# TSultanov/cfd-demo

Hardware: AMD Instinct MI355X
Metric: cell-updates/s (Poisson iter) + ms/timestep, 4096² grid, 1/2/4/8 GPU (higher is better)
Workload: dtype f32

## Files before the change

### cfd-demo_amd/csrc/cfd_correct.h

```cpp
#pragma once
#include "cfd_device.h"

namespace cfd {
namespace {

template <int SP>
__device__ __forceinline__ float u_corr(const Geom &g, float us, float pr, float pw, float dt, int i) {
    return i >= g.nx - 7 ? us - sdiv<SP>(dt * (pr - pw), g.dx, g.r_dx)
                         : us - dt * sdiv<SP>(pr - pw, g.dx, g.r_dx);
}

template <int SP>
__device__ __forceinline__ float v_corr(const Geom &g, float vs, float pt, float pb, float dt) {
    return vs - dt * sdiv<SP>(pt - pb, g.dy, g.r_dy);
}
template <int SP>
__device__ __forceinline__ void v_corr4(const Geom &g, const float4 &vs, const float4 &pt,
                                        const float4 &pb, float dt, float4 &o) {
    o.x = v_corr<SP>(g, vs.x, pt.x, pb.x, dt);
    o.y = v_corr<SP>(g, vs.y, pt.y, pb.y, dt);
    o.z = v_corr<SP>(g, vs.z, pt.z, pb.z, dt);
    o.w = v_corr<SP>(g, vs.w, pt.w, pb.w, dt);
}

__device__ __forceinline__ float4 add4(float4 a, const float4 &b) {
    a.x = a.x + b.x;
    a.y = a.y + b.y;
    a.z = a.z + b.z;
    a.w = a.w + b.w;
    return a;
}

__device__ __forceinline__ void publish_step_maxima(const Fields &f, int bid, float du, float dv,
                                                    float mu, float mv) {
    __shared__ float red[kBlock / 64][4];
    du = wave_max(du);
    dv = wave_max(dv);
    mu = wave_max(mu);
    mv = wave_max(mv);
    const int wv = threadIdx.x >> 6;
    if ((threadIdx.x & 63) == 0) {
        red[wv][0] = du;
        red[wv][1] = dv;
        red[wv][2] = mu;
        red[wv][3] = mv;
    }
    __syncthreads();
    if (threadIdx.x < 4) {
        float r = 0.f;
#pragma unroll
        for (int w = 0; w < kBlock / 64; ++w) r = fmaxf(r, red[w][threadIdx.x]);
        publish_max(f.red_slots + (size_t)threadIdx.x * kResSlots * kResStride, bid, r);
    }
}

__device__ __forceinline__ void publish_sums_m0_bound(const Geom &g, Ctl *c, uint32_t pm) {
    const uint32_t thr = __float_as_uint(kSumsPLim * g.dx_sq);
    raise_bits_bound(&c->sums_m0, pm, thr);
    if (blockIdx.x == 0 && threadIdx.x == 0) {
        atomicMax(&c->sums_m0, thr);
        c->sums_rm = 0u;
        c->sums_state = 1u;
    }
}

}
}
```

### cfd-demo_amd/csrc/cfd_correct.hip

```cpp
#include "cfd_correct.h"

namespace cfd {
namespace {


template <int SP>
__global__ __launch_bounds__(kBlock) void k_corrector(Geom g, Fields f, int pass,
                                                      float dt_override, int nbx) {
    Ctl *c = f.ctl;
    if (pass_off(c, pass)) return;
    const int bid = xcd_block(g);
    const int i = (bid % nbx) * kBlock + (int)threadIdx.x;
    const int lj = bid / nbx;
    const int nx = g.nx, W = nx + 1;
    if (i > nx) return;
    const float dt = dt_of(c, dt_override);
    const float *__restrict__ pp = c->cur ? f.pp[1] : f.pp[0];
    const int j = g.j0 + lj;
    if (lj < g.nyl && i >= 1 && i <= nx - 1) {
        const float p_right = pp[(long)lj * nx + i];
        const float p_left = pp[(long)lj * nx + i - 1];
        const long k = (long)lj * W + i;
        f.u[k] = u_corr<SP>(g, f.u_star[k], p_right, p_left, dt, i);
    }
    if (i < nx && j >= 1 && j <= g.ny - 1) {
        const float p_top = pp[(long)lj * nx + i];
        const float p_bottom = pp[(long)(lj - 1) * nx + i];
        const long k = (long)lj * nx + i;
        f.v[k] = v_corr<SP>(g, f.v_star[k], p_top, p_bottom, dt);
    }
    if (i < nx && lj < g.nyl) {
        const long k = (long)lj * nx + i;
        f.p[k] = f.p[k] + pp[k];
    }
}

template <int SP>
__global__ __launch_bounds__(kBlock) void k_corrector4(Geom g, Fields f, int pass,
                                                       float dt_override, int nbx) {
    Ctl *c = f.ctl;
    if (pass_off(c, pass)) return;
    const int bid = xcd_block(g);
    const int i0 = 4 * ((bid % nbx) * kBlock + (int)threadIdx.x);
    const int lj = bid / nbx;
    const int nx = g.nx, W = nx + 1;
    if (i0 >= nx) return;
    const float dt = dt_of(c, dt_override);
    const float *__restrict__ pp = c->cur ? f.pp[1] : f.pp[0];
    const int j = g.j0 + lj;
    const long kc = (long)lj * nx + i0;
    float4 pc = {0.f, 0.f, 0.f, 0.f};
    if (lj < g.nyl) {
        pc = *reinterpret_cast<const float4 *>(pp + kc);
        const float pl = i0 > 0 ? pp[kc - 1] : 0.0f;
        const float pr[4] = {pc.x, pc.y, pc.z, pc.w};
        const float pw[4] = {pl, pc.x, pc.y, pc.z};
        const long ku = (long)lj * W + i0;
#pragma unroll
        for (int q = 0; q < 4; ++q) {
            const int i = i0 + q;
            if (i < 1 || i > nx - 1) continue;
            f.u[ku + q] = u_corr<SP>(g, f.u_star[ku + q], pr[q], pw[q], dt, i);
        }
    }
    if (j >= 1 && j <= g.ny - 1) {
        const float4 pt = lj < g.nyl ? pc : *reinterpret_cast<const float4 *>(pp + kc);
        const float4 pb = *reinterpret_cast<const float4 *>(pp + kc - nx);
        const float4 vs = *reinterpret_cast<const float4 *>(f.v_star + kc);
        float4 o;
        v_corr4<SP>(g, vs, pt, pb, dt, o);
        *reinterpret_cast<float4 *>(f.v + kc) = o;
    }
    if (lj < g.nyl)
        *reinterpret_cast<float4 *>(f.p + kc) = add4(*reinterpret_cast<const float4 *>(f.p + kc), pc);
}

template <int SP, int ROWS>
__global__ __launch_bounds__(kBlock) void k_correct_head4(Geom g, Fields f, int pass,
                                                          float dt_override, int nbx, int has_next) {
    Ctl *c = f.ctl;
    if (pass_off(c, pass)) return;
    const bool head = has_next && c->go[pass + 1] != 0;
    const bool odd = pass & 1;
    const float *__restrict__ in_u = odd ? f.u : f.u_star;
    const float *__restrict__ in_v = odd ? f.v : f.v_star;
    float *__restrict__ out_u = odd ? f.u_star : f.u;
    float *__restrict__ out_v = odd ? f.v_star : f.v;
    const int bid = xcd_block(g);
    const int i0 = 4 * ((bid % nbx) * kBlock + (int)threadIdx.x);
    const int nx = g.nx, W = nx + 1, nyl = g.nyl;
    if (i0 >= nx) return;
    const float dt = dt_of(c, dt_override);
    const float *__restrict__ pp = c->cur ? f.pp[1] : f.pp[0];
    auto v_row = [&](int r, const float4 &pt, bool *hit) -> float4 {
        const int jr = g.j0 + r;
        const long k = (long)r * nx + i0;
        *hit = jr >= 1 && jr <= g.ny - 1;
        if (!*hit) return *reinterpret_cast<const float4 *>(f.v + k);
        const float4 pb = *reinterpret_cast<const float4 *>(pp + k - nx);
        const float4 vs = *reinterpret_cast<const float4 *>(in_v + k);
        float4 o;
        v_corr4<SP>(g, vs, pt, pb, dt, o);
        return o;
    };
    const int lr0 = (bid / nbx) * ROWS - kGhostUV, lr1 = min(lr0 + ROWS, nyl + 1 + kGhostUV);
    bool carry = false;
    float4 p_next = {0.f, 0.f, 0.f, 0.f}, v_next = {0.f, 0.f, 0.f, 0.f};
    struct HRow {
        float4 pld, pt, vsn, pv;
        f4u iu;
        float iu4, plv, p4v;
    };
    HRow cur, nxt;
    bool have = false;
    auto load_hrow = [&](int r, HRow &h) {
        const long kc = (long)r * nx + i0, ku = (long)r * W + i0;
        h.pld = *reinterpret_cast<const float4 *>(pp + kc);
        h.plv = pp[kc - (i0 > 0 ? 1 : 0)];
        h.p4v = pp[kc + (i0 + 4 < nx ? 4 : 3)];
        h.iu = *reinterpret_cast<const f4u *>(in_u + ku);
        h.iu4 = in_u[ku + 4];
        h.pt = *reinterpret_cast<const float4 *>(pp + kc + nx);
        const int jr = g.j0 + r + 1;
        h.vsn = *reinterpret_cast<const float4 *>((jr >= 1 && jr <= g.ny - 1 ? in_v : f.v) + kc + nx);
        h.pv = *reinterpret_cast<const float4 *>(f.p + kc);
    };
    for (int lr = lr0; lr < lr1; ++lr) {
        const long kc = (long)lr * nx + i0, ku = (long)lr * W + i0;
        const bool owned = lr >= 0 && lr < nyl;
        if (odd && (!head || !owned)) {
            *reinterpret_cast<float4 *>(f.v_star + kc) = *reinterpret_cast<const float4 *>(f.v + kc);
            if (lr < nyl + kGhostUV) {
                const float *__restrict__ ur = f.u + ku;
                float *__restrict__ us = f.u_star + ku;
                *reinterpret_cast<f4u *>(us) = *reinterpret_cast<const f4u *>(ur);
                if (i0 + 4 == nx) us[4] = ur[4];
            }
        }
        if (!owned && (head || lr != nyl)) {
            carry = false;
            have = false;
            continue;
        }
        if (!head) {
            float4 pc = {0.f, 0.f, 0.f, 0.f};
            if (owned) {
                pc = *reinterpret_cast<const float4 *>(pp + kc);
                const float pl = i0 > 0 ? pp[kc - 1] : 0.0f;
                const float pr[4] = {pc.x, pc.y, pc.z, pc.w};
                const float pw[4] = {pl, pc.x, pc.y, pc.z};
#pragma unroll
                for (int q = 0; q < 4; ++q) {
                    const int i = i0 + q;
                    if (i < 1 || i > nx - 1) continue;
                    f.u[ku + q] = u_corr<SP>(g, in_u[ku + q], pr[q], pw[q], dt, i);
                }
            }
            bool hit;
            const float4 o = v_row(lr, owned ? pc : *reinterpret_cast<const float4 *>(pp + kc), &hit);
            if (hit) *reinterpret_cast<float4 *>(f.v + kc) = o;
            if (owned)
                *reinterpret_cast<float4 *>(f.p + kc) = add4(*reinterpret_cast<const float4 *>(f.p + kc), pc);
            carry = false;
            have = false;
            continue;
        }
        if (!have) load_hrow(lr, cur);
        const bool pf = ROWS > 1 && lr + 1 < lr1 && lr + 1 < nyl;
        if (pf) load_hrow(lr + 1, nxt);
        const float4 pc = carry ? p_next : cur.pld;
        const float pl = i0 > 0 ? cur.plv : 0.0f;
        const float p4 = i0 + 4 < nx ? cur.p4v : 0.0f;
        const float pr[5] = {pc.x, pc.y, pc.z, pc.w, p4};
        const float pw[5] = {pl, pc.x, pc.y, pc.z, pc.w};
        float un[5];
        const float iuq[5] = {cur.iu.x, cur.iu.y, cur.iu.z, cur.iu.w, cur.iu4};
#pragma unroll
        for (int q = 0; q < 5; ++q) un[q] = u_corr<SP>(g, iuq[q], pr[q], pw[q], dt, i0 + q);
        if (i0 == 0) un[0] = f.u[ku];
        if (i0 + 4 == nx) un[4] = f.u[ku + 4];
        *reinterpret_cast<f4u *>(out_u + ku) = (f4u){un[0], un[1], un[2], un[3]};
        if (i0 + 4 == nx) out_u[ku + 4] = un[4];
        bool hit;
        const float4 vlo = carry ? v_next : v_row(lr, pc, &hit);
        const float4 pt = cur.pt;
        float4 vhi = cur.vsn;
        {
            const int jr = g.j0 + lr + 1;
            if (jr >= 1 && jr <= g.ny - 1) v_corr4<SP>(g, cur.vsn, pt, pc, dt, vhi);
        }
        *reinterpret_cast<float4 *>(out_v + kc) = vlo;
        *reinterpret_cast<float4 *>(f.p + kc) = add4(cur.pv, pc);
        *reinterpret_cast<float4 *>(f.rhs + kc) = div4<SP>(g, un[0], un[1], un[2], un[3], un[4], vlo, vhi, dt);
        if (pf) cur = nxt;
        have = pf;
        carry = ROWS > 1;
        p_next = pt;
        v_next = vhi;
    }
}


template <int SP>
__device__ __forceinline__ float cf_u_face(const Geom &g, float inlet, float dt, int i, int j,
                                           float ustar, float p_right, float p_left) {
    const int nx = g.nx;
    if (j == 0) return 0.0f;
    if (j == g.ny - 1) return (g.bc_kind == 1 && i > 0 && i < nx) ? inlet : 0.0f;
    if (i == 0) return g.bc_kind == 0 ? inlet_value(g, inlet, j) : 0.0f;
    if (i == nx) return g.bc_kind == 0 ? u_corr<SP>(g, ustar, p_right, p_left, dt, nx) : 0.0f;
    return u_corr<SP>(g, ustar, p_right, p_left, dt, i);
}

template <int SP>
__device__ __forceinline__ void cf4_row(const Geom &g, const Fields &f, const float *__restrict__ pp,
                                        float inlet, float dt, int i0, int lj, const float4 &pc,
                                        const float4 &pb, float &du, float &dv, float &mu,
                                        float &mv, bool &bad) {
    const int nx = g.nx, W = nx + 1;
    const int j = g.j0 + lj;
    const long rp = (long)lj * nx + i0;
    const bool vrow = (j != 0 && j != g.ny);
    if (lj < g.nyl) {
        const long k = (long)lj * W + i0;
        const float pl = (i0 > 0) ? pp[rp - 1] : 0.0f;
        const f4u su = *reinterpret_cast<const f4u *>(f.u_star + k);
        const float s0 = su.x, s1 = su.y, s2 = su.z, s3 = su.w;
        float n0 = cf_u_face<SP>(g, inlet, dt, i0, j, s0, pc.x, pl);
        float n1 = cf_u_face<SP>(g, inlet, dt, i0 + 1, j, s1, pc.y, pc.x);
        float n2 = cf_u_face<SP>(g, inlet, dt, i0 + 2, j, s2, pc.z, pc.y);
        float n3 = cf_u_face<SP>(g, inlet, dt, i0 + 3, j, s3, pc.w, pc.z);
        if (f.n_obs > 0) {
            if (f.mask_u[k] & 2) n0 = 0.0f;
            if (f.mask_u[k + 1] & 2) n1 = 0.0f;
            if (f.mask_u[k + 2] & 2) n2 = 0.0f;
            if (f.mask_u[k + 3] & 2) n3 = 0.0f;
        }
        const f4u uo = *reinterpret_cast<const f4u *>(f.u + k);
        const float o0 = uo.x, o1 = uo.y, o2 = uo.z, o3 = uo.w;
        *reinterpret_cast<f4u *>(f.u + k) = (f4u){n0, n1, n2, n3};
        du = fmaxf(fmaxf(fmaxf(du, fabsf(n0 - o0)), fmaxf(fabsf(n1 - o1), fabsf(n2 - o2))),
                   fabsf(n3 - o3));
        mu = fmaxf(fmaxf(fmaxf(mu, fabsf(n0)), fmaxf(fabsf(n1), fabsf(n2))), fabsf(n3));
        bad |= nonfinite(n0) || nonfinite(n1) || nonfinite(n2) || nonfinite(n3);
        if (i0 + 4 == nx) {
            float n4 = cf_u_face<SP>(g, inlet, dt, nx, j, s3, pc.w, pc.z);
            if (f.n_obs > 0 && (f.mask_u[k + 4] & 2)) n4 = 0.0f;
            const float o4 = f.u[k + 4];
            f.u[k + 4] = n4;
            du = fmaxf(du, fabsf(n4 - o4));
            mu = fmaxf(mu, fabsf(n4));
            bad |= nonfinite(n4);
        }
    }
    float4 nv = make_float4(0.f, 0.f, 0.f, 0.f);
    if (vrow) v_corr4<SP>(g, *reinterpret_cast<const float4 *>(f.v_star + rp), pc, pb, dt, nv);
    if (f.n_obs > 0) {
        if (f.mask_v[rp] & 2) nv.x = 0.0f;
        if (f.mask_v[rp + 1] & 2) nv.y = 0.0f;
        if (f.mask_v[rp + 2] & 2) nv.z = 0.0f;
        if (f.mask_v[rp + 3] & 2) nv.w = 0.0f;
    }
    const float4 ov = *reinterpret_cast<const float4 *>(f.v + rp);
    *reinterpret_cast<float4 *>(f.v + rp) = nv;
    dv = fmaxf(fmaxf(fmaxf(dv, fabsf(nv.x - ov.x)), fmaxf(fabsf(nv.y - ov.y), fabsf(nv.z - ov.z))),
               fabsf(nv.w - ov.w));
    mv = fmaxf(fmaxf(fmaxf(mv, fabsf(nv.x)), fmaxf(fabsf(nv.y), fabsf(nv.z))), fabsf(nv.w));
    bad |= nonfinite(nv.x) || nonfinite(nv.y) || nonfinite(nv.z) || nonfinite(nv.w);
    if (lj < g.nyl)
        *reinterpret_cast<float4 *>(f.p + rp) = add4(*reinterpret_cast<const float4 *>(f.p + rp), pc);
}

#ifndef CFD_CF_ROWS
#define CFD_CF_ROWS 16
#endif
constexpr int kCfRows = CFD_CF_ROWS;
template <int SP, int ROWS>
__global__ __launch_bounds__(kBlock) void k_correct_finish4m(Geom g, Fields f, float dt_override,
                                                             int nbx) {
    Ctl *c = f.ctl;
    const int nx = g.nx;
    float du = 0.f, dv = 0.f, mu = 0.f, mv = 0.f;
    uint32_t pm = 0u;
    bool bad = false;
    const int bid = xcd_block(g);
    const int i0 = 4 * ((bid % nbx) * kBlock + (int)threadIdx.x);
    const int l0 = (bid / nbx) * ROWS, l1 = min(l0 + ROWS, g.nyl + 1);
    const float dt = dt_of(c, dt_override);
    const float inlet = c->inlet;
    const float *__restrict__ pp = c->cur ? f.pp[1] : f.pp[0];
    if (i0 < nx) {
        float4 pb = make_float4(0.f, 0.f, 0.f, 0.f);
        {
            const int j = g.j0 + l0;
            if (j != 0 && j != g.ny) pb = *reinterpret_cast<const float4 *>(pp + (long)(l0 - 1) * nx + i0);
        }
        for (int lj = l0; lj < l1; ++lj) {
            const int j = g.j0 + lj;
            const bool vrow = (j != 0 && j != g.ny);
            float4 pc = make_float4(0.f, 0.f, 0.f, 0.f);
            if (lj < g.nyl || vrow) pc = *reinterpret_cast<const float4 *>(pp + (long)lj * nx + i0);
            cf4_row<SP>(g, f, pp, inlet, dt, i0, lj, pc, vrow ? pb : make_float4(0.f, 0.f, 0.f, 0.f),
                        du, dv, mu, mv, bad);
            if (f.sums_track && lj < g.nyl)
                pm = max(max(pm, max(abs_bits(pc.x), abs_bits(pc.y))), max(abs_bits(pc.z), abs_bits(pc.w)));
            pb = pc;
        }
    }
    flag_nonfinite(c, bad);
    if (f.sums_track) publish_sums_m0_bound(g, c, pm);
    publish_step_maxima(f, bid, du, dv, mu, mv);
}

__global__ __launch_bounds__(kBlock) void k_publish_sums_m0(Geom g, Fields f) {
    Ctl *c = f.ctl;
    const float *__restrict__ pp = c->cur ? f.pp[1] : f.pp[0];
    const size_t n = (size_t)g.nx * (size_t)g.nyl;
    uint32_t pm = 0u;
    for (size_t k = (size_t)blockIdx.x * kBlock + threadIdx.x; k < n; k += (size_t)gridDim.x * kBlock)
        pm = max(pm, abs_bits(pp[k]));
    publish_sums_m0_bound(g, c, pm);
}

int cf_rows(const Geom &g, int nbx, int nrows) {
    return (long)nbx * cdiv(nrows, kCfRows) >= 2L * g.n_cu ? kCfRows : 1;
}

}


void launch_corrector(const Geom &g, const Fields &f, int pass, float dt_override, bool vec,
                      hipStream_t s) {
    if (vec && g.nx % 4 == 0 && aligned16(f.v) && aligned16(f.v_star) && aligned16(f.p) &&
        aligned16(f.pp[0]) && aligned16(f.pp[1])) {
        const int nbx4 = cdiv(g.nx / 4, kBlock);
        if (g.sp_pow2)
            hipLaunchKernelGGL(k_corrector4<1>, dim3(nbx4 * (g.nyl + 1)), dim3(kBlock), 0, s, g, f,
                               pass, dt_override, nbx4);
        else
            hipLaunchKernelGGL(k_corrector4<0>, dim3(nbx4 * (g.nyl + 1)), dim3(kBlock), 0, s, g, f,
                               pass, dt_override, nbx4);
        return;
    }
    const int nbx = cdiv(g.nx + 1, kBlock);
    if (g.sp_pow2)
        hipLaunchKernelGGL(k_corrector<1>, dim3(nbx * (g.nyl + 1)), dim3(kBlock), 0, s, g, f, pass,
                           dt_override, nbx);
    else
        hipLaunchKernelGGL(k_corrector<0>, dim3(nbx * (g.nyl + 1)), dim3(kBlock), 0, s, g, f, pass,
                           dt_override, nbx);
}

bool correct_head_ok(const Geom &g, const Fields &f) {
    return g.nx % 4 == 0 && aligned16(f.v) && aligned16(f.v_star) && aligned16(f.p) &&
           aligned16(f.pp[0]) && aligned16(f.pp[1]) && aligned16(f.rhs);
}

void launch_correct_head(const Geom &g, const Fields &f, int pass, float dt_override, bool has_next,
                         hipStream_t s) {
    const int nbx4 = cdiv(g.nx / 4, kBlock);
    const int hn = has_next ? 1 : 0;
    const int nrows = g.nyl + 1 + 2 * kGhostUV;
    const int rows = cf_rows(g, nbx4, nrows);
    const dim3 grid(nbx4 * cdiv(nrows, rows));
#define CFD_LAUNCH_CH(SPV, RW)                                                                    \
    hipLaunchKernelGGL((k_correct_head4<SPV, RW>), grid, dim3(kBlock), 0, s, g, f, pass, dt_override, \
                       nbx4, hn)
    if (rows == kCfRows) {
        if (g.sp_pow2) CFD_LAUNCH_CH(1, kCfRows); else CFD_LAUNCH_CH(0, kCfRows);
    } else {
        if (g.sp_pow2) CFD_LAUNCH_CH(1, 1); else CFD_LAUNCH_CH(0, 1);
    }
#undef CFD_LAUNCH_CH
}

void launch_correct_finish(const Geom &g, const Fields &f, float dt_override, hipStream_t s) {
    const int nbx = cdiv(g.nx / 4, kBlock);
    const int rows = cf_rows(g, nbx, g.nyl + 1);
    const dim3 grid(nbx * cdiv(g.nyl + 1, rows));
#define CFD_LAUNCH_CF(SPV, RW)                                                                     \
    hipLaunchKernelGGL((k_correct_finish4m<SPV, RW>), grid, dim3(kBlock), 0, s, g, f, dt_override, nbx)
    if (rows == kCfRows) {
        if (g.sp_pow2) CFD_LAUNCH_CF(1, kCfRows); else CFD_LAUNCH_CF(0, kCfRows);
    } else {
        if (g.sp_pow2) CFD_LAUNCH_CF(1, 1); else CFD_LAUNCH_CF(0, 1);
    }
#undef CFD_LAUNCH_CF
}

void launch_publish_sums_m0(const Geom &g, const Fields &f, hipStream_t s) {
    const size_t n = (size_t)g.nx * (size_t)g.nyl;
    hipLaunchKernelGGL(k_publish_sums_m0, dim3(copy_grid(n)), dim3(kBlock), 0, s, g, f);
}

}
```

### cfd-demo_amd/csrc/cfd_internal.h

```cpp
#pragma once
#include <hip/hip_runtime.h>
#include <stdint.h>

#include <type_traits>

#include "../../include/cfd.h"

namespace cfd {

template <class Fn>
auto with_fastdiv(int fastdiv, Fn &&f) {
    if (fastdiv == 1) return f(std::integral_constant<int, 1>{});
    if (fastdiv == 2) return f(std::integral_constant<int, 2>{});
    return f(std::integral_constant<int, 0>{});
}

constexpr int kGhostUV = 2;
constexpr float kSumsPLim = 0x1p122f, kSumsRLim = 0x1p112f;
constexpr int kMaxSweeps = 4096;
constexpr int kMaxPasses = 64;

constexpr int kResSlots = 32;
constexpr int kResStride = 16;
constexpr int kPersistFlagStride = 16;
constexpr int kPersistHeadLines = 21;
constexpr int kPersistBlockBits = 10;
static_assert((1 << kPersistBlockBits) > kMaxSweeps / 8, "persistent flag layout");
constexpr int kPersistMaxGroups = 16384;
constexpr size_t kPersistWords = (size_t)(kPersistMaxGroups + kPersistHeadLines) * kPersistFlagStride;
constexpr size_t kSlotWords = (size_t)(kMaxSweeps + 16) * kResSlots * kResStride + kPersistWords;

struct Ctl {
    float dt;
    float time;
    uint32_t step;
    float inlet;
    int32_t cur;
    uint32_t n_exec_last;
    float last_p;
    float res_u, res_v;
    uint32_t red[7];
    uint32_t nonfinite_step;
    uint32_t vis[2];
    uint32_t sums_state;
    uint64_t sweeps_total;
    int32_t spec_stop, spec_redo, spec_launch, spec_launches;
    uint32_t sums_launches;
    uint32_t sums_m0, sums_rm;
    int32_t go[kMaxPasses + 1];
    uint32_t err[kMaxSweeps];
    double last_p64;
};

constexpr int kRes64Stride = 8;
constexpr size_t kRes64Words = (size_t)kMaxSweeps * kResSlots * kRes64Stride;

struct Geom {
    int32_t nx, ny;
    int32_t j0, nyl;
    int32_t hg;
    float dx, dy, nu, ly;
    float target_inlet;
    int32_t scheme, profile, bc_kind;
    int32_t tol_enabled;
    float p_tol;
    int32_t jacobi_iters;
    float dx_sq, dy_sq, denom;
    float r_dx_sq, r_dy_sq, r_denom;
    int32_t fastdiv;
    int32_t tb_rows;
    int32_t tb_bpc;
    int32_t n_cu;
    int32_t tb_kind;
    int32_t xcd_remap;
    float r_dx, r_dy, r_dxx, r_dyy;
    int32_t sp_pow2;
    int32_t pred_div;
    int32_t res_div;
};

struct Fields {
    float *u, *v, *u_old, *v_old, *u_star, *v_star;
    float *p, *rhs;
    float *pp[2];
    const uint8_t *mask_u, *mask_v;
    const int32_t *obs;
    uint32_t *err_slots;
    uint32_t *red_slots;
    uint32_t *vis_slots;
    int32_t n_obs;
    int32_t any_pmask;
    size_t u_alloc, v_alloc;
    float *u_alloc_base, *v_alloc_base, *u_old_base, *v_old_base, *u_star_base, *v_star_base;
    Ctl *ctl;
    uint32_t *host_nonfinite;
    uint32_t *host_progress;
    uint32_t *persist;
    int32_t sums_track;
};

inline bool aligned16(const void *p) { return ((uintptr_t)p & 15u) == 0; }

void launch_step_begin(const Geom &g, const Fields &f, int copy, hipStream_t s);
void launch_copy_star(const Geom &g, const Fields &f, int pass, hipStream_t s);
void launch_copy_star_div(const Geom &g, const Fields &f, int pass, float dt_override,
                          hipStream_t s);
void launch_u_predictor(const Geom &g, const Fields &f, float dt_override, hipStream_t s);
void launch_v_predictor(const Geom &g, const Fields &f, float dt_override, hipStream_t s);
void launch_predict(const Geom &g, const Fields &f, float dt_override, bool vec, hipStream_t s);
bool predict_march_ok(const Geom &g, const Fields &f);
void launch_predict_march(const Geom &g, const Fields &f, float dt_override, hipStream_t s,
                          bool set_inlet = false, int row_lo = 0, int row_hi = -1);
void launch_divergence(const Geom &g, const Fields &f, int pass, float dt_override,
                       hipStream_t s);
void launch_jacobi_sweep(const Geom &g, const Fields &f, int pass, int it, int row_lo,
                         int row_hi, int res, hipStream_t s);
void launch_jacobi_block(const Geom &g, const Fields &f, int pass, int it, int par, int T,
                         int out_lo, int out_hi, int res, hipStream_t s);
bool launch_jacobi_persist(const Geom &g, const Fields &f, int pass, int par0, int nblk,
                           int out_lo, int out_hi, uint32_t epoch, int res_it, hipStream_t s);
void lds_geometry8(const Geom &g, int out_lo, int out_hi, bool persist, int *pad, int *occ, int *nwc,
                   int *nseg);
void launch_tb1(const Geom &g, const Fields &f, int T, int pass, int it, int par, int out_lo,
                int out_hi, uint32_t *res_slots, hipStream_t s);
void launch_pipe(const Geom &g, const Fields &f, int T, int pass, int it, int par, int out_lo,
                 int out_hi, uint32_t *res_slots, hipStream_t s);
bool launch_lds_persist8(const Geom &g, const Fields &f, int pass, int par0, int nblk, int out_lo,
                         int out_hi, uint32_t epoch, uint32_t *rs, hipStream_t s);
void launch_lds(const Geom &g, const Fields &f, int T, int pass, int it, int par, int out_lo,
                int out_hi, uint32_t *res_slots, hipStream_t s, int mode = 0, int lag = 0);
void launch_jacobi_spec(const Geom &g, const Fields &f, int pass, int it, int par, int T,
                        int out_lo, int out_hi, hipStream_t s, int lag = 0);
void launch_spec_check(const Geom &g, const Fields &f, int pass, int it, int T, int par,
                       hipStream_t s);
bool launch_jacobi_resident(const Geom &g, const Fields &f, int pass, int iters, int fin,
                            int check_break, hipStream_t s);
bool jacobi_resident_geometry(const Geom &g, int *br, int *bc, int *tiles, int *wgs);
void launch_spec_align(const Geom &g, const Fields &f, int pass, int n, hipStream_t s);
void launch_jacobi_redo(const Geom &g, const Fields &f, int pass, int out_lo, int out_hi,
                        hipStream_t s, int last_it = 0, int last_par = 0, int last_T = 0);
void launch_fold_slots(uint32_t *dst, uint32_t *slots, int n, hipStream_t s);
void launch_vis_field(const Geom &g, const Fields &f, int mode, float *out, uint32_t *slots,
                      hipStream_t s);
void launch_vis_color(const Geom &g, const Fields &f, int mode, const float *field, uint32_t *px,
                      const uint32_t *keys, int has_cyl, float cx, float cy, float radius,
                      hipStream_t s);
void launch_verify_division(float c, float r, unsigned long long *dev_counts, hipStream_t s);
void launch_finalize_solve(const Geom &g, const Fields &f, int pass, int iters, int check_break,
                           int flips, hipStream_t s, int exact_flips = 0);

struct SorConst {
    double dx2, dy2, denom;
    double r_dx2, r_dy2, r_denom;
    int32_t fast;
};
struct MgLevel {
    float *a, *b, *rhs, *r;
    int32_t nx, ny;
    double dx2, dy2, denom;
    double r_dx2, r_dy2, r_denom;
    int32_t fast;
    int32_t ys, ye;
    int32_t lo, hi;
};
constexpr int kMgMaxLevels = 40;
void launch_sor_color(float *pp, const float *rhs, int nx, int ny, const SorConst &k, int color,
                      Ctl *ctl, uint32_t *err_slots, int pass, int it, int tol, float p_tol, int res,
                      hipStream_t s);
bool sor_fused_ok(int nx, int nrows);
void launch_sor_fused(float *pa, float *pb, const float *rhs, int nx, int ny, const SorConst &k,
                      Ctl *ctl, uint32_t *err_slots, int pass, int it, int tol, float p_tol, int res,
                      int row_lo, int row_hi, int j0, int lo_clamp, int hi_clamp, hipStream_t s);
void launch_fill_zero(float *p, size_t n, const Ctl *ctl, int pass, hipStream_t s);
size_t sor_lex_words(int iters, int ny);
hipError_t launch_sor_lex(float *pa, float *pb, const float *rhs, int nx, int ny, const SorConst &k,
                          Ctl *ctl, uint32_t *pol, uint32_t *exitw, uint32_t *host_fail, int pass,
                          int iters, int tol, float p_tol, int n_cu, int *launches, hipStream_t s,
                          unsigned long long *res64 = nullptr);
void launch_jacobi_script(float *pa, float *pb, const float *rhs, int nx, int ny, const SorConst &k,
                          Ctl *ctl, uint32_t *err_slots, int pass, int it, int tol, float p_tol,
                          int res, hipStream_t s, unsigned long long *res64 = nullptr);
void launch_publish_f64(const Fields &f, unsigned long long *res64, int pass, int iters, int z_lo,
                        int to_n, hipStream_t s);
void launch_mg_smooth(const MgLevel &L, const float *src, float *dst, const Ctl *ctl, int pass,
                      hipStream_t s);
void launch_mg_smooth5(const MgLevel &L, const float *src, float *dst, const Ctl *ctl, int pass,
                       hipStream_t s);
bool mg_smooth_wave_form();
void launch_mg_prolong_smooth5(const MgLevel &Cl, const float *e, const MgLevel &L, const float *src,
                               float *dst, const Ctl *ctl, int pass, hipStream_t s);
void launch_mg_smooth5_residual(const MgLevel &L, const float *src, float *dst, const Ctl *ctl,
                                int pass, hipStream_t s);
void launch_mg_residual(const MgLevel &L, const float *p, const Ctl *ctl, int pass, hipStream_t s);
void launch_mg_restrict(const MgLevel &F, const MgLevel &Cl, const Ctl *ctl, int pass, hipStream_t s);
void launch_mg_prolong_add(const MgLevel &Cl, const float *e, const MgLevel &F, float *p,
                           const Ctl *ctl, int pass, hipStream_t s);
void launch_mg_tail(const MgLevel *dev_levels, int s_level, int coarsest, float *a0, float *b0,
                    int fast, const Ctl *ctl, int pass, hipStream_t s);
void launch_mg_final_residual(const MgLevel &L, const float *p, uint32_t *slots, const Ctl *ctl,
                              int pass, hipStream_t s, unsigned long long *res64 = nullptr);
void launch_boundary(const Geom &g, const Fields &f, hipStream_t s);
void launch_step_reduce(const Geom &g, const Fields &f, hipStream_t s);
void launch_step_finalize(const Geom &g, const Fields &f, hipStream_t s);
void launch_abort_to_red(const Fields &f, hipStream_t s);
void launch_abort_from_red(const Fields &f, hipStream_t s);

void launch_corrector(const Geom &g, const Fields &f, int pass, float dt_override, bool vec,
                      hipStream_t s);
void launch_correct_finish(const Geom &g, const Fields &f, float dt_override, hipStream_t s);
void launch_publish_sums_m0(const Geom &g, const Fields &f, hipStream_t s);
bool correct_head_ok(const Geom &g, const Fields &f);
void launch_correct_head(const Geom &g, const Fields &f, int pass, float dt_override, bool has_next,
                         hipStream_t s);

constexpr int kTrcBlock = 256;
struct TrcCtl {
    uint32_t count;
    uint32_t overflow;
    uint32_t cur;
    uint32_t n_prev, src, total, do_inject;
    uint32_t ticket;
};
struct Tracers {
    double *x0, *y0, *i0, *x1, *y1, *i1;
    TrcCtl *tc;
    uint32_t *tile_cnt, *tile_off;
    uint32_t cap;
    uint32_t interval;
    double dx, dy, lx, ly;
};
void launch_trc_step(const Geom &g, const Fields &f, const Tracers &t, int grid, bool in_step,
                     double dt, hipStream_t s);
void launch_trc_inject(const Geom &g, const Tracers &t, hipStream_t s);
void launch_trc_density(const Geom &g, const Tracers &t, int grid, uint32_t *counts, hipStream_t s);

struct ScriptStep {
    double dx, dy, dxx, dyy, nu, dt;
    double r_dx, r_dy, r_dxx, r_dyy;
    const int32_t *obs_u, *obs_v;
    const float *inlet;
    int32_t fast;
};
bool script_step_ok(const Geom &g, const Fields &f);
void launch_script_predict(const Geom &g, const Fields &f, const ScriptStep &k, int scheme,
                           hipStream_t s);
void launch_script_correct(const Geom &g, const Fields &f, const ScriptStep &k, hipStream_t s);

constexpr int kScrRedStride = 8;
constexpr int kScrRedPmax = 3 * kResSlots * kScrRedStride;
constexpr int kScrRedWords = kScrRedPmax + kScrRedStride;
void launch_script_begin(const Fields &f, float *u_prev, float *u_old, float *v_prev, float *v_old,
                         long nu, long nv, int extrapolate, hipStream_t s);
void launch_script_pmax(const Fields &f, unsigned long long *red, hipStream_t s);
void launch_script_pmax64(const Fields &f, unsigned long long *red, hipStream_t s);
void launch_script_end(const Fields &f, float *u_prev, const float *u_old, float *v_prev,
                       const float *v_old, long nu, long nv, unsigned long long *red, hipStream_t s);

constexpr int kJacRowsPerWave = 16;
constexpr int kMaxTemporal = 8;
constexpr int kJacWavesPerBlock = 4;

}
```

### cfd-demo_amd/csrc/cfd_model.h

```cpp
#pragma once

#include <hip/hip_runtime.h>
#include <rccl/rccl.h>

#include <climits>
#include <cmath>
#include <condition_variable>
#include <cstdint>
#include <cstdlib>
#include <functional>
#include <initializer_list>
#include <mutex>
#include <string>
#include <utility>
#include <vector>

#include "../../include/cfd.h"
#include "cfd_internal.h"
#include "slab_plan.h"

namespace cfd {

int fail(int code, const std::string &msg);

inline int env_int(const char *name, int def) {
    const char *e = getenv(name);
    return e ? atoi(e) : def;
}
inline long env_long(const char *name, long def) {
    const char *e = getenv(name);
    return e ? atol(e) : def;
}
inline bool env_flag(const char *name, bool def) {
    const char *e = getenv(name);
    return e ? atoi(e) != 0 : def;
}
inline double env_double(const char *name, double def) {
    const char *e = getenv(name);
    return e ? atof(e) : def;
}
constexpr int kEnvUnset = INT_MIN;

inline bool exact_pow2(double c) {
    int e;
    return c > 0.0 && std::isfinite(c) && std::frexp(c, &e) == 0.5 && std::isnormal(1.0 / c);
}

inline size_t round4(size_t n) { return (n + 3) & ~size_t(3); }

}

#define HIP_TRY(expr)                                                                      \
    do {                                                                                   \
        hipError_t e_ = (expr);                                                            \
        if (e_ != hipSuccess)                                                              \
            return cfd::fail(CFD_EHIP, std::string(#expr) + ": " + hipGetErrorString(e_)); \
    } while (0)

#define RCCL_TRY(expr)                                                                     \
    do {                                                                                   \
        ncclResult_t r_ = (expr);                                                          \
        if (r_ != ncclSuccess)                                                             \
            return cfd::fail(CFD_ERCCL, std::string(#expr) + ": " + ncclGetErrorString(r_)); \
    } while (0)

#define RCCL_OP(expr)                                                                      \
    do {                                                                                   \
        int rc_ = settle((expr), #expr);                                                   \
        if (rc_) return rc_;                                                               \
    } while (0)

struct LocalHub {
    int n = 0;
    std::mutex mu;
    std::condition_variable cv;
    int arrived = 0;
    uint64_t gen = 0;
    std::vector<cfd_model *> members;
    void barrier() {
        std::unique_lock<std::mutex> lk(mu);
        const uint64_t my = gen;
        if (++arrived == n) {
            arrived = 0;
            ++gen;
            cv.notify_all();
        } else {
            cv.wait(lk, [&] { return gen != my; });
        }
    }
};

enum FieldId { FLD_U = 0, FLD_V, FLD_PP0, FLD_PP1, FLD_RHS };

struct PersistGate {
    std::mutex mu;
    hipEvent_t ev = nullptr;
    hipStream_t last = nullptr;
};

struct cfd_options {
    bool sor_fused = true;
    bool mg_partition = true;
    bool spec = true;
    bool spec_lag = true;
    bool spec_slabs = true;
    int persist = -1;
    bool persist_sharded = false;
    bool persist_gate = false;
    int resident = -1;
    bool copy_div = true;
    bool pred_vec = true;
    bool corr_vec = true;
    bool corr_head = true;
    bool graph = false;
    bool ckpt = true;
    int fastdiv = cfd::kEnvUnset;
    int resident_div = cfd::kEnvUnset;
    int pred_div = cfd::kEnvUnset;
    int tb_kind = cfd::kEnvUnset;
    int temporal = cfd::kEnvUnset;
    int tb_rows = cfd::kEnvUnset;
    int tb_bpc = cfd::kEnvUnset;
    int xcd_remap = cfd::kEnvUnset;
    double rccl_timeout_s = 300.0;
};

struct cfd_model {
    int device = 0;
    cfd_grid grid{};
    cfd_params params{};
    cfd_options opt{};
    cfd::Geom g{};
    cfd::Fields f{};

    hipStream_t stream = nullptr;
    hipStream_t cstream = nullptr;
    hipEvent_t ev_ov0 = nullptr, ev_ov1 = nullptr, ev_rhs = nullptr, ev_uv = nullptr;
    static constexpr bool overlap = true;

    float *u_all = nullptr, *v_all = nullptr, *uo_all = nullptr, *vo_all = nullptr;
    float *us_all = nullptr, *vs_all = nullptr;
    float *p = nullptr, *rhs = nullptr, *pp_all[2] = {nullptr, nullptr};
    uint8_t *mask_u = nullptr, *mask_v = nullptr;
    int32_t *obs = nullptr;
    cfd::Ctl *ctl = nullptr;
    uint32_t *slots = nullptr;
    float *vis_buf = nullptr;
    uint32_t *h_nonfinite = nullptr;
    std::vector<uint8_t> h_mask_u, h_mask_v;
    std::vector<uint8_t> dmask_u, dmask_v;

    int n_ranks = 1, rank = 0;
    uint64_t j0 = 0, j1 = 0;
    ncclComm_t comm = nullptr;
    LocalHub *hub = nullptr;
    bool comm_aborted = false;
    uint64_t comm_calls = 0;
    bool pp_ghosts_shallow = false;

    int host_cur = 0;
    int t_max = cfd::kMaxTemporal;
    static constexpr int kResRing = 8;
    uint32_t *h_res = nullptr;
    hipEvent_t ev_res[kResRing] = {};
    static constexpr int kSpecRing = 4;
    uint32_t *h_spec = nullptr;
    hipEvent_t ev_spec[kSpecRing] = {};
    bool spec_converged = false;
    bool persist_on = true;
    uint32_t persist_epoch = 0;
    int last_persist_blocks = 0;
    bool capturing = false;
    static constexpr long kResidentAutoCells = 1l << 21;
    bool resident_off = false;
    uint64_t resident_solves = 0;
    bool last_abort_resident = false;
    bool merge_res_allreduce = false;

    uint32_t *lex_pol = nullptr, *lex_exit = nullptr;
    size_t lex_words = 0;
    cfd_script_options sopt{};
    unsigned long long *res64 = nullptr;
    bool p64_valid = false;
    std::vector<cfd::MgLevel> mg;
    cfd::MgLevel *mg_dev = nullptr;
    float *mg_pool = nullptr;
    int mg_tail = 0;
    int mg_P = 0;
    static constexpr int kMgGhost = 8;
    static constexpr int kSmT5 = 5;
    struct MgX {
        int l, which, depth;
    };

    bool step_begin_folded = false;
    bool uv_async = false;
    bool stepped = false;
    hipGraphExec_t step_graph = nullptr;
    int graph_cur_delta = 0;
    int graph_steps = 4;
    struct CkSeg {
        void *ptr;
        size_t bytes;
    };
    std::vector<CkSeg> ck_segs;
    char *ck_pool = nullptr;
    size_t ck_bytes = 0;
    bool ck_open = false;
    int ck_host_cur = 0;
    bool ck_shallow = false;
    std::vector<std::function<int()>> ck_replay;
    uint64_t recoveries = 0;

    hipEvent_t ev_step0 = nullptr, ev_step1 = nullptr, ev_prof0 = nullptr, ev_prof1 = nullptr;
    bool timing = false;
    std::vector<hipEvent_t> ev_pool;
    size_t ev_next = 0;
    std::vector<std::pair<hipEvent_t, hipEvent_t>> solve_events;
    std::vector<hipEvent_t> step_events;
    uint64_t timed_sweeps = 0, timed_steps = 0, timed_launches = 0;
    double timed_step_ms = 0.0;
    bool timing_phases = false;
    std::vector<std::pair<hipEvent_t, hipEvent_t>> phase_events[3];
    double phase_ms[3] = {0.0, 0.0, 0.0};
    uint64_t phase_count[3] = {0, 0, 0};

    cfd::Tracers trc{};
    char *trc_pool = nullptr;
    size_t trc_bytes = 0;
    int trc_grid = 0;
    uint32_t *trc_dens = nullptr;
    char *scr_pool = nullptr;
    cfd::ScriptStep scr{};
    std::vector<float> scr_inlet_h;
    double scr_inlet_v = 0.0;
    int scr_inlet_profile = -1;

    char *su_pool = nullptr;
    float *su_uprev = nullptr, *su_vprev = nullptr, *su_uold = nullptr, *su_vold = nullptr;
    unsigned long long *su_red = nullptr, *su_h = nullptr;
    bool su_begun = false, su_bad = false;
    bool su_failed = false;
    bool su_dt_set = false;
    double su_dt = 0.0;
    int32_t su_substeps = 5;
    uint64_t su_steps = 0;
    double su_inlet = 0.0;
    double su_pmax64 = 0.0;

    bool sharded() const { return n_ranks > 1; }
    size_t u_rows_alloc() const { return (size_t)g.nyl + 2 * cfd::kGhostUV; }
    size_t v_rows_alloc() const { return (size_t)g.nyl + 1 + 2 * cfd::kGhostUV; }

    struct HaloX {
        int id, kind, depth;
    };
    float *field_ptr(int id);
    size_t field_pitch(int id) const { return id == FLD_U ? (size_t)g.nx + 1 : (size_t)g.nx; }
    int exchange_group(std::initializer_list<HaloX> items, hipStream_t st);
    int exchange_ops(int id, int kind, int depth, hipStream_t st);
    int exchange_local(int id, int kind, int depth, hipStream_t st);
    int exchange(int id, int kind, int depth, hipStream_t st = nullptr) {
        return exchange_group({{id, kind, depth}}, st);
    }
    int exchange_uv(hipStream_t st = nullptr) {
        return exchange_group({{FLD_U, cfd::HALO_U, 2}, {FLD_V, cfd::HALO_V, 2}}, st);
    }
    int exchange_pp(int buf, int rows, hipStream_t st = nullptr) {
        return exchange(buf ? FLD_PP1 : FLD_PP0, cfd::HALO_PP, rows, st);
    }
    int exchange_rhs_pp(int rhs_rows, int buf, int pp_rows) {
        return exchange_group({{FLD_RHS, cfd::HALO_PP, rhs_rows},
                               {buf ? FLD_PP1 : FLD_PP0, cfd::HALO_PP, pp_rows}}, nullptr);
    }
    int allreduce_max_u32(uint32_t *dev, size_t n);
    int settle(ncclResult_t r, const char *what);
    int wait_done(hipEvent_t ev);

    bool spec_mode() const;
    bool resident_mode() const;
    bool spec_slab_ok() const;
    bool host_driven() const;
    int gate_wait(PersistGate &gate, bool always);
    int launch_persist(int pass, int par0, int nblk, int lo, int hi, int res_it, bool *done);
    int enqueue_solve(int pass);
    int enqueue_jacobi_single(int pass);
    int enqueue_jacobi_slabs(int pass);
    int enqueue_spec_slabs(int pass);
    int enqueue_solve_host_driven(float *residual_out);

    static void level_consts(double dx, double dy, double *dx2, double *dy2, double *denom,
                             double *r, int32_t *fast);
    cfd::SorConst sor_consts() const;
    int enqueue_sor(int pass);
    int enqueue_sor_sharded(const cfd::SorConst &k, int pass, float *residual_out, hipEvent_t e0);
    int enqueue_sor_sharded_deep(const cfd::SorConst &k, int pass, hipEvent_t e0);
    int enqueue_sor_lex(int pass);
    int enqueue_jacobi_script(int pass);
    unsigned long long *res64_on() const { return sopt.residual_f64 && !sharded() ? res64 : nullptr; }
    int clear_res64();
    void mg_rows(int l, int r, int *j0o, int *j1o) const;
    int mg_partition_levels(const std::vector<std::pair<int, int>> &dims, int tail) const;
    int mg_build();
    int gather_rhs();
    int mg_exchange(std::initializer_list<MgX> items);
    int mg_allgather_rhs(int l);
    int enqueue_mg_partitioned(int pass, float *residual_out, hipEvent_t e0);
    int enqueue_mg(int pass, float *residual_out = nullptr);

    hipEvent_t take_event();
    hipEvent_t phase_mark(int ph, bool end, hipStream_t st = nullptr);
    void begin_solve_timing(int pass, hipEvent_t *e0);
    void end_solve_timing(hipEvent_t e0, uint64_t sweeps, uint64_t launches);
    void pass_head(int pass, float dt_override);
    int enqueue_piso(float dt_override, bool finish = false);
    int enqueue_update(bool rec_step = true);
    bool graph_ok() const;
    void drop_graph();
    int update_graph(int n);
    int abort_allreduce();
    int sync();
    int read_ctl(cfd::Ctl *out);
    int persist_timeout_check(bool at_sync);
    bool ckpt_needed() const;
    int ck_begin();
    void ck_record(std::function<int()> fn);
    void ck_commit();
    int ck_drop_pool();
    int recover();
    int invalidate_sums();
    int clear_abort_words();

    int trc_release();
    bool scr_in_obstacle(double x, double y) const;
    int script_build();
    int script_prepare(const cfd_script_step *s, cfd::ScriptStep *out);
    int script_substep(const cfd_script_step *s);

    int su_alloc();
    int su_update(const cfd_script_config *c, cfd_script_report *out);

    void destroy();
};

namespace cfd {
cfd_options read_options();
int validate(const cfd_grid *grid, const cfd_params *p);
int validate_sharded(const cfd_model *m, const cfd_params *p);
void apply_params(cfd_model *m, const cfd_params *p);
void set_sums_track(cfd_model *m);
int create_model(const cfd_grid *grid, const cfd_params *params, int device, int n_ranks, int rank,
                 const void *uid, LocalHub *hub, cfd_model **out);
int script_check(cfd_model *m, const cfd_script_step *s);
int comm_init(cfd_model *m, const ncclUniqueId &id, int n_ranks, int rank);
PersistGate &persist_gate(int device);
}
```

### cfd-demo_amd/csrc/cfd_model_abi.hip

```cpp
#include <cstddef>
#include <cstdio>
#include <cstring>

#include "cfd_model.h"

using namespace cfd;

namespace {
thread_local std::string g_last_error;
}

int cfd::fail(int code, const std::string &msg) {
    g_last_error = msg;
    return code;
}

extern "C" {

const char *cfd_last_error(void) { return g_last_error.c_str(); }
void cfdrt_set_error(const char *msg) { g_last_error = msg ? msg : ""; }
int cfdrt_check_params(const cfd_model *m, const cfd_params *p) {
    if (!m) return fail(CFD_EINVAL, "null model");
    int rc = validate(&m->grid, p);
    if (rc) return rc;
    return validate_sharded(m, p);
}

int cfd_get_config(const cfd_model *m, cfd_grid *grid, cfd_params *params) {
    if (!m) return fail(CFD_EINVAL, "null model");
    if (grid) *grid = m->grid;
    if (params) *params = m->params;
    return 0;
}
int cfd_abi_version(void) { return CFD_ABI_VERSION; }

void cfd_default_params(cfd_params *o) {
    if (!o) return;
    o->dt = 0.005f;
    o->viscosity = 0.000001f;
    o->target_inlet_velocity = 1.0f;
    o->velocity_scheme = CFD_SCHEME_FIRST_ORDER;
    o->inlet_profile = CFD_INLET_UNIFORM;
    o->pressure_solver = CFD_SOLVER_JACOBI;
    o->jacobi_iters = 50;
    o->corrector_passes = 20;
    o->tol_enabled = 1;
    o->p_tol = 1e-4f;
    o->bc_kind = CFD_BC_CHANNEL;
}

void cfd_default_grid(cfd_grid *o) {
    if (!o) return;
    o->nx = 800;
    o->ny = 264;
    o->lx = 30.0f;
    o->ly = 10.0f;
    o->has_cylinder = 1;
    o->cylinder_x = 30.0f / 4.0f;
    o->cylinder_y = 10.0f / 2.0f;
    o->cylinder_radius = 0.75f;
}

int cfd_create(const cfd_grid *grid, const cfd_params *params, int device_ordinal, cfd_model **out) {
    return create_model(grid, params, device_ordinal, 1, 0, nullptr, nullptr, out);
}

int cfd_create_sharded(const cfd_grid *grid, const cfd_params *params, int device_ordinal,
                       int n_ranks, int rank, const void *uid, cfd_model **out) {
    if (n_ranks > 1 && !uid) return fail(CFD_EINVAL, "null rccl unique id");
    return create_model(grid, params, device_ordinal, n_ranks, rank, uid, nullptr, out);
}

int cfd_create_sharded_local(const cfd_grid *grid, const cfd_params *params, int device_ordinal,
                             int n_ranks, int rank, void *hub, cfd_model **out) {
    if (!hub) return fail(CFD_EINVAL, "null local hub");
    return create_model(grid, params, device_ordinal, n_ranks, rank, nullptr,
                         static_cast<LocalHub *>(hub), out);
}

int cfd_device_count(int *n_out) {
    if (!n_out) return fail(CFD_EINVAL, "null out");
    *n_out = 0;
    int n = 0;
    const hipError_t e = hipGetDeviceCount(&n);
    if (e != hipSuccess && e != hipErrorNoDevice)
        return fail(CFD_EHIP, std::string("hipGetDeviceCount: ") + hipGetErrorString(e));
    *n_out = e == hipSuccess ? n : 0;
    return 0;
}

int cfd_get_comm_size(const cfd_model *m, int *n_out) {
    if (!m || !n_out) return fail(CFD_EINVAL, "null model or out");
    if (m->hub) {
        *n_out = m->hub->n;
    } else if (m->comm) {
        int n = 0;
        RCCL_TRY(ncclCommCount(m->comm, &n));
        *n_out = n;
    } else if (m->n_ranks > 1) {
        return fail(CFD_ERCCL, "the RCCL communicator was aborted after an earlier failure");
    } else {
        *n_out = 1;
    }
    return 0;
}

int cfd_get_slab(const cfd_model *m, uint64_t *j0, uint64_t *j1) {
    if (!m) return fail(CFD_EINVAL, "null model");
    if (j0) *j0 = m->j0;
    if (j1) *j1 = m->j1;
    return 0;
}

int cfd_update(cfd_model *m) { return cfd_update_n(m, 1); }

int cfd_update_n(cfd_model *m, int n) {
    if (!m) return fail(CFD_EINVAL, "null model");
    HIP_TRY(hipSetDevice(m->device));
    if (int rc = m->persist_timeout_check(false)) return rc;
    if (const uint32_t bad = *(volatile uint32_t *)m->h_nonfinite)
        return fail(CFD_ENONFINITE, "non-finite velocity (NaN/Inf) after step " + std::to_string(bad) +
                                        "; cfd_set_state clears it");
    if (n <= 0) return 0;
    if (int rc = m->ck_begin()) return rc;
    m->ck_record([m, n]() {
        for (int k = 0; k < n; ++k)
            if (int rc = m->enqueue_update(k == n - 1)) return rc;
        return 0;
    });
    if (m->timing) {
        hipEvent_t e0 = m->take_event();
        HIP_TRY(hipEventRecord(e0, m->stream));
        m->step_events.push_back(e0);
    }
    int rc = 0;
    if (m->graph_ok()) {
        rc = m->update_graph(n);
    } else {
        for (int k = 0; k < n && !rc; ++k) rc = m->enqueue_update(k == n - 1);
    }
    if (m->timing) {
        hipEvent_t e1 = m->take_event();
        HIP_TRY(hipEventRecord(e1, m->stream));
        m->step_events.push_back(e1);
    }
    return rc;
}

int cfd_piso_step(cfd_model *m, float dt_sub) {
    if (!m) return fail(CFD_EINVAL, "null model");
    HIP_TRY(hipSetDevice(m->device));
    if (int rc = m->invalidate_sums()) return rc;
    if (int rc = m->ck_begin()) return rc;
    auto run = [m, dt_sub]() {
        int rc = m->exchange_uv();
        if (!rc) rc = m->enqueue_piso(dt_sub);
        return rc ? rc : m->abort_allreduce();
    };
    m->ck_record(run);
    return run();
}

int cfd_pressure_solve(cfd_model *m, float *residual_out) {
    if (!m) return fail(CFD_EINVAL, "null model");
    HIP_TRY(hipSetDevice(m->device));
    int rc;
    if ((rc = m->invalidate_sums())) return rc;
    if (m->host_driven()) {
        return m->enqueue_solve_host_driven(residual_out);
    }
    if ((rc = m->ck_begin())) return rc;
    auto run = [m]() {
        int rc2 = m->enqueue_solve(-1);
        return rc2 ? rc2 : m->abort_allreduce();
    };
    m->ck_record(run);
    rc = run();
    if (rc) return rc;
    Ctl c;
    rc = m->read_ctl(&c);
    if (rc) return rc;
    if (residual_out) *residual_out = c.last_p;
    return 0;
}

int cfd_run_phase(cfd_model *m, int phase, float dt_sub) {
    if (!m) return fail(CFD_EINVAL, "null model");
    HIP_TRY(hipSetDevice(m->device));
    if (int rc = m->invalidate_sums()) return rc;
    switch (phase) {
    case CFD_PHASE_U_PREDICTOR: {
        int rc = m->exchange_uv();
        if (rc) return rc;
        launch_u_predictor(m->g, m->f, dt_sub, m->stream);
        break;
    }
    case CFD_PHASE_V_PREDICTOR: {
        int rc = m->exchange_uv();
        if (rc) return rc;
        launch_v_predictor(m->g, m->f, dt_sub, m->stream);
        break;
    }
    case CFD_PHASE_DIVERGENCE: launch_divergence(m->g, m->f, -1, dt_sub, m->stream); break;
    case CFD_PHASE_CORRECTOR: launch_corrector(m->g, m->f, -1, dt_sub, m->opt.corr_vec, m->stream); break;
    case CFD_PHASE_BOUNDARY: launch_boundary(m->g, m->f, m->stream); break;
    default: return fail(CFD_EINVAL, "unknown phase");
    }
    HIP_TRY(hipGetLastError());
    return m->sync();
}

int cfd_set_params(cfd_model *m, const cfd_params *p) {
    if (!m) return fail(CFD_EINVAL, "null model");
    int rc = validate(&m->grid, p);
    if (rc) return rc;
    rc = validate_sharded(m, p);
    if (rc) return rc;
    rc = m->sync();
    if (rc) return rc;
    m->drop_graph();
    {
        Ctl c;
        rc = m->read_ctl(&c);
        if (rc) return rc;
        m->host_cur = c.cur;
    }
    apply_params(m, p);
    set_sums_track(m);
    rc = m->invalidate_sums();
    if (rc) return rc;
    HIP_TRY(hipMemcpy(&m->ctl->dt, &p->dt, 4, hipMemcpyHostToDevice));
    return 0;
}

int cfd_get_snapshot(cfd_model *m, float *u, float *v, float *p, float *dt_out) {
    if (!m) return fail(CFD_EINVAL, "null model");
    int rc = m->sync();
    if (rc) return rc;
    const size_t W = (size_t)m->g.nx + 1, nx = (size_t)m->g.nx, nyl = (size_t)m->g.nyl;
    if (u) HIP_TRY(hipMemcpy(u, m->f.u, nyl * W * 4, hipMemcpyDeviceToHost));
    if (v) HIP_TRY(hipMemcpy(v, m->f.v, (nyl + 1) * nx * 4, hipMemcpyDeviceToHost));
    if (p) HIP_TRY(hipMemcpy(p, m->f.p, nyl * nx * 4, hipMemcpyDeviceToHost));
    if (dt_out) HIP_TRY(hipMemcpy(dt_out, &m->ctl->dt, 4, hipMemcpyDeviceToHost));
    return 0;
}

namespace {

float decode_key(uint32_t k, bool is_min) {
    if (is_min) {
        if (!k) return INFINITY;
        k = ~k;
    } else if (!k) {
        return -INFINITY;
    }
    const uint32_t b = (k & 0x80000000u) ? (k & 0x7FFFFFFFu) : ~k;
    float x;
    std::memcpy(&x, &b, 4);
    return x;
}

int render_common(cfd_model *m, int mode, bool field, void *host_out, float *min_max_out) {
    if (!m) return fail(CFD_EINVAL, "null model");
    if (mode < CFD_VIS_PRESSURE || mode > CFD_VIS_VORTICITY)
        return fail(CFD_EINVAL, "unknown visualisation mode");
    HIP_TRY(hipSetDevice(m->device));
    const size_t n = (size_t)m->g.nx * (size_t)m->g.nyl;
    if (!m->vis_buf) HIP_TRY(hipMalloc((void **)&m->vis_buf, n * 4));
    if (mode == CFD_VIS_VORTICITY) {
        int rc = m->exchange_uv();
        if (rc) return rc;
    }
    Fields &f = m->f;
    launch_vis_field(m->g, f, mode, field ? m->vis_buf : nullptr, f.vis_slots, m->stream);
    launch_fold_slots(f.ctl->vis, f.vis_slots, 2, m->stream);
    int rc = m->allreduce_max_u32(f.ctl->vis, 2);
    if (rc) return rc;
    const cfd_grid &gr = m->grid;
    if (!field && host_out)
        launch_vis_color(m->g, f, mode, nullptr, (uint32_t *)m->vis_buf, f.ctl->vis,
                         gr.has_cylinder, gr.cylinder_x, gr.cylinder_y, gr.cylinder_radius,
                         m->stream);
    HIP_TRY(hipGetLastError());
    uint32_t keys[2] = {0u, 0u};
    HIP_TRY(hipMemcpyAsync(keys, f.ctl->vis, 8, hipMemcpyDeviceToHost, m->stream));
    HIP_TRY(hipMemsetAsync(f.ctl->vis, 0, 8, m->stream));
    if (host_out) HIP_TRY(hipMemcpyAsync(host_out, m->vis_buf, n * 4, hipMemcpyDeviceToHost, m->stream));
    if (int rc2 = m->wait_done(nullptr)) return rc2;
    if (min_max_out) {
        min_max_out[0] = decode_key(keys[1], true);
        min_max_out[1] = decode_key(keys[0], false);
    }
    return 0;
}

}

int cfd_render(cfd_model *m, int mode, uint8_t *rgba, float *min_max_out) {
    return render_common(m, mode, false, rgba, min_max_out);
}

int cfd_derive_field(cfd_model *m, int mode, float *out, float *min_max_out) {
    return render_common(m, mode, true, out, min_max_out);
}

int cfd_get_residuals(cfd_model *m, cfd_residuals *out) {
    if (!m || !out) return fail(CFD_EINVAL, "null argument");
    Ctl c;
    int rc = m->read_ctl(&c);
    if (rc) return rc;
    out->simulation_step = c.step;
    out->simulation_time = c.time;
    out->dt = c.dt;
    out->p = c.last_p;
    out->u = c.res_u;
    out->v = c.res_v;
    out->piso_substeps = 1;
    out->jacobi_sweeps_total = c.sweeps_total;
    float ms = 0.f;
    if (m->stepped && hipEventElapsedTime(&ms, m->ev_step0, m->ev_step1) == hipSuccess)
        out->step_time_s = ms * 1e-3;
    else
        out->step_time_s = 0.0;
    if (c.nonfinite_step)
        return fail(CFD_ENONFINITE, "non-finite velocity (NaN/Inf) after step " +
                                        std::to_string(c.nonfinite_step));
    return 0;
}

int cfd_get_state(cfd_model *m, cfd_state *st) {
    if (!m || !st) return fail(CFD_EINVAL, "null argument");
    Ctl c;
    int rc = m->read_ctl(&c);
    if (rc) return rc;
    const size_t W = (size_t)m->g.nx + 1, nx = (size_t)m->g.nx, nyl = (size_t)m->g.nyl;
    if (st->u) HIP_TRY(hipMemcpy(st->u, m->f.u, nyl * W * 4, hipMemcpyDeviceToHost));
    if (st->v) HIP_TRY(hipMemcpy(st->v, m->f.v, (nyl + 1) * nx * 4, hipMemcpyDeviceToHost));
    if (st->p) HIP_TRY(hipMemcpy(st->p, m->f.p, nyl * nx * 4, hipMemcpyDeviceToHost));
    if (st->u_star) HIP_TRY(hipMemcpy(st->u_star, m->f.u_star, nyl * W * 4, hipMemcpyDeviceToHost));
    if (st->v_star) HIP_TRY(hipMemcpy(st->v_star, m->f.v_star, (nyl + 1) * nx * 4, hipMemcpyDeviceToHost));
    if (st->p_prime) HIP_TRY(hipMemcpy(st->p_prime, m->f.pp[c.cur], nyl * nx * 4, hipMemcpyDeviceToHost));
    if (st->rhs) HIP_TRY(hipMemcpy(st->rhs, m->f.rhs, nyl * nx * 4, hipMemcpyDeviceToHost));
    st->dt = c.dt;
    st->simulation_time = c.time;
    st->simulation_step = c.step;
    st->last_p_residual = c.last_p;
    st->last_u_residual = c.res_u;
    st->last_v_residual = c.res_v;
    st->jacobi_sweeps_total = c.sweeps_total;
    return 0;
}

int cfd_set_state(cfd_model *m, const cfd_state *st) {
    if (!m || !st) return fail(CFD_EINVAL, "null argument");
    Ctl c;
    int rc = m->read_ctl(&c);
    if (rc) return rc;
    const size_t W = (size_t)m->g.nx + 1, nx = (size_t)m->g.nx, nyl = (size_t)m->g.nyl;
    if (st->u) HIP_TRY(hipMemcpy(m->f.u, st->u, nyl * W * 4, hipMemcpyHostToDevice));
    if (st->v) HIP_TRY(hipMemcpy(m->f.v, st->v, (nyl + 1) * nx * 4, hipMemcpyHostToDevice));
    if (st->p) HIP_TRY(hipMemcpy(m->f.p, st->p, nyl * nx * 4, hipMemcpyHostToDevice));
    if (st->u_star) HIP_TRY(hipMemcpy(m->f.u_star, st->u_star, nyl * W * 4, hipMemcpyHostToDevice));
    if (st->v_star) HIP_TRY(hipMemcpy(m->f.v_star, st->v_star, (nyl + 1) * nx * 4, hipMemcpyHostToDevice));
    if (st->p_prime) HIP_TRY(hipMemcpy(m->f.pp[c.cur], st->p_prime, nyl * nx * 4, hipMemcpyHostToDevice));
    if (st->rhs) HIP_TRY(hipMemcpy(m->f.rhs, st->rhs, nyl * nx * 4, hipMemcpyHostToDevice));
    c.dt = st->dt;
    c.time = st->simulation_time;
    c.step = (uint32_t)st->simulation_step;
    c.last_p = st->last_p_residual;
    c.res_u = st->last_u_residual;
    c.res_v = st->last_v_residual;
    c.sweeps_total = st->jacobi_sweeps_total;
    c.nonfinite_step = 0;
    c.red[4] = 0;
    c.red[6] = 0;
    c.sums_state = 0;
    c.sums_m0 = 0;
    rc = m->clear_abort_words();
    if (rc) return rc;
    HIP_TRY(hipMemcpy(m->f.ctl, &c, offsetof(Ctl, go), hipMemcpyHostToDevice));
    HIP_TRY(hipMemset(&m->f.ctl->last_p64, 0, 8));
    m->p64_valid = false;
    *(volatile uint32_t *)m->h_nonfinite = 0u;
    m->host_cur = c.cur;
    rc = m->exchange_uv();
    if (rc) return rc;
    rc = m->exchange_pp(c.cur, m->g.hg);
    if (rc) return rc;
    return m->sync();
}

int cfd_script_set_options(cfd_model *m, const cfd_script_options *o) {
    if (!m || !o) return fail(CFD_EINVAL, "null argument");
    if (m->sharded()) return fail(CFD_EINVAL, "script options need a single-domain model");
    if ((o->residual_f64 != 0 && o->residual_f64 != 1) ||
        (o->residual_scaling != 0 && o->residual_scaling != 1))
        return fail(CFD_EINVAL, "script options take 0 or 1");
    if (int rc = m->sync()) return rc;
    m->drop_graph();
    cfd_script_options n = *o;
    if (n.residual_scaling) n.residual_f64 = 1;
    if (n.residual_f64 && !m->res64) {
        HIP_TRY(hipMalloc((void **)&m->res64, kRes64Words * 8));
        if (int rc = m->clear_res64()) return rc;
    }
    if (!n.residual_f64) {
        m->p64_valid = false;
        if (m->res64) HIP_TRY(hipFree(m->res64));
        m->res64 = nullptr;
    }
    m->sopt = n;
    return 0;
}

int cfd_script_get_options(const cfd_model *m, cfd_script_options *o) {
    if (!m || !o) return fail(CFD_EINVAL, "null argument");
    *o = m->sopt;
    return 0;
}

int cfd_get_p_residual_f64(cfd_model *m, double *last, double *step_max) {
    if (!m) return fail(CFD_EINVAL, "null model");
    if (!m->sopt.residual_f64) return fail(CFD_ESTATE, "residual_f64 is off (cfd_script_set_options)");
    if (!m->p64_valid)
        return fail(CFD_ESTATE, "no solve has published a double residual: none has run since the option "
                                "was set or the state was replaced, or the last one was solver 0 or 1");
    if (int rc = m->sync()) return rc;
    if (last) HIP_TRY(hipMemcpy(last, &m->f.ctl->last_p64, 8, hipMemcpyDeviceToHost));
    if (step_max) *step_max = m->su_pmax64;
    return 0;
}

int cfd_get_masks(cfd_model *m, uint8_t *mask_u, uint8_t *mask_v) {
    if (!m) return fail(CFD_EINVAL, "null model");
    if (mask_u) std::memcpy(mask_u, m->h_mask_u.data(), m->h_mask_u.size());
    if (mask_v) std::memcpy(mask_v, m->h_mask_v.data(), m->h_mask_v.size());
    return 0;
}

int cfd_synchronize(cfd_model *m) {
    if (!m) return fail(CFD_EINVAL, "null model");
    return m->sync();
}

int cfd_profile_sweeps(cfd_model *m, int n_sweeps, double *avg_ms_out) {
    if (!m) return fail(CFD_EINVAL, "null model");
    if (n_sweeps < 1 || n_sweeps > kMaxSweeps) return fail(CFD_EINVAL, "n_sweeps out of range");
    HIP_TRY(hipSetDevice(m->device));
    if (int rc = m->invalidate_sums()) return rc;
    const int lo = std::max(0, 1 - (int)m->j0), hi = std::min(m->g.nyl, (int)m->g.ny - 1 - (int)m->j0);
    hipEvent_t a = m->ev_prof0, b = m->ev_prof1;
    Geom g = m->g;
    g.tol_enabled = 0;
    HIP_TRY(hipEventRecord(a, m->stream));
    for (int it = 0; it < n_sweeps; ++it)
        launch_jacobi_sweep(g, m->f, -1, it, lo, hi, it == n_sweeps - 1, m->stream);
    HIP_TRY(hipEventRecord(b, m->stream));
    launch_finalize_solve(g, m->f, -1, n_sweeps, 0, n_sweeps, m->stream);
    HIP_TRY(hipGetLastError());
    m->host_cur = (m->host_cur + n_sweeps) & 1;
    m->pp_ghosts_shallow = m->sharded();
    int rc = m->sync();
    if (rc) return rc;
    float ms = 0.f;
    HIP_TRY(hipEventElapsedTime(&ms, a, b));
    if (avg_ms_out) *avg_ms_out = ms / n_sweeps;
    return 0;
}

int cfd_timing_begin(cfd_model *m) {
    if (!m) return fail(CFD_EINVAL, "null model");
    int rc = m->sync();
    if (rc) return rc;
    m->timing = true;
    m->ev_next = 0;
    m->solve_events.clear();
    m->step_events.clear();
    for (auto &pe : m->phase_events) pe.clear();
    m->timed_sweeps = 0;
    m->timed_launches = 0;
    m->timed_steps = 0;
    return 0;
}

int cfd_timing_end(cfd_model *m, double *solve_ms, uint64_t *sweeps, double *step_ms, uint64_t *steps) {
    if (!m) return fail(CFD_EINVAL, "null model");
    int rc = m->sync();
    if (rc) return rc;
    double s_ms = 0.0, t_ms = 0.0;
    for (auto &pr : m->solve_events) {
        float ms = 0.f;
        HIP_TRY(hipEventElapsedTime(&ms, pr.first, pr.second));
        s_ms += ms;
    }
    for (size_t k = 0; k + 1 < m->step_events.size(); k += 2) {
        float ms = 0.f;
        HIP_TRY(hipEventElapsedTime(&ms, m->step_events[k], m->step_events[k + 1]));
        t_ms += ms;
    }
    for (int ph = 0; ph < 3; ++ph) {
        m->phase_ms[ph] = 0.0;
        m->phase_count[ph] = 0;
        for (auto &pr : m->phase_events[ph]) {
            float ms = 0.f;
            if (!pr.second) continue;
            HIP_TRY(hipEventElapsedTime(&ms, pr.first, pr.second));
            m->phase_ms[ph] += ms;
            ++m->phase_count[ph];
        }
        m->phase_events[ph].clear();
    }
    if (solve_ms) *solve_ms = s_ms;
    if (sweeps) *sweeps = m->timed_sweeps;
    if (step_ms) *step_ms = t_ms;
    if (steps) *steps = m->timed_steps;
    m->timing = false;
    m->ev_next = 0;
    m->solve_events.clear();
    m->step_events.clear();
    return 0;
}

int cfd_timing_phases(cfd_model *m, int on) {
    if (!m) return fail(CFD_EINVAL, "null model");
    m->timing_phases = on != 0;
    return 0;
}

int cfd_timing_phase_ms(const cfd_model *m, double *predict_ms, double *finish_ms) {
    if (!m) return fail(CFD_EINVAL, "null model");
    if (predict_ms) *predict_ms = m->phase_ms[0];
    if (finish_ms) *finish_ms = m->phase_ms[1];
    return 0;
}

int cfd_timing_exchange_ms(const cfd_model *m, double *exchange_ms, uint64_t *exchanges) {
    if (!m) return fail(CFD_EINVAL, "null model");
    if (exchange_ms) *exchange_ms = m->phase_ms[2];
    if (exchanges) *exchanges = m->phase_count[2];
    return 0;
}

int cfd_get_halo_depth(const cfd_model *m) { return m ? m->g.hg : 0; }

int cfd_get_kernel_config(const cfd_model *m, int *fastdiv, int *temporal) {
    if (!m) return fail(CFD_EINVAL, "null model");
    if (fastdiv) *fastdiv = m->g.fastdiv;
    if (temporal) *temporal = m->spec_mode() ? kMaxTemporal : m->g.tol_enabled ? 1 : m->t_max;
    return 0;
}

int cfd_get_jacobi_kernel(const cfd_model *m, int *kind, char *name, size_t name_len) {
    if (!m) return fail(CFD_EINVAL, "null model");
    const bool spec = m->spec_mode();
    const bool resident = m->resident_mode();
    const int T = spec ? kMaxTemporal : m->g.tol_enabled ? 1 : m->t_max;
    const int k = resident ? 6 : spec ? 5 : T <= 1 ? 0 : m->g.tb_kind;
    if (kind) *kind = k;
    if (name && name_len) {
        char buf[96];
        if (resident)
            snprintf(buf, sizeof buf, "k_jacobi_resident<%d>", m->g.res_div);
        else if (spec)
            snprintf(buf, sizeof buf, "k_jacobi_lds<%d, %d, 2>", T, m->g.fastdiv);
        else if (k == 0)
            snprintf(buf, sizeof buf, "k_jacobi<%d, %d>", kJacRowsPerWave, m->g.fastdiv);
        else if (k == 1)
            snprintf(buf, sizeof buf, "k_jacobi_tb<%d, %d>", T, m->g.fastdiv);
        else if (k == 5)
            snprintf(buf, sizeof buf, "k_jacobi_lds<%d, %d, 0>", T, m->g.fastdiv);
        else
            snprintf(buf, sizeof buf, "k_jacobi_pipe<%d, %d>", T, m->g.fastdiv);
        snprintf(name, name_len, "%s", buf);
    }
    return 0;
}

int cfd_get_jacobi_geometry(const cfd_model *m, int persist, int *lds_pad, int *wgs_per_cu,
                            int *wave_cols, int *segments) {
    if (!m) return fail(CFD_EINVAL, "null model");
    if (hipSetDevice(m->device) != hipSuccess) return fail(CFD_EHIP, "hipSetDevice");
    int T, lo, hi, exch;
    plan_block((int)m->j0, m->g.nyl, m->g.ny, m->sharded() ? m->g.hg : 0, 0, 8,
               std::max(8, m->params.jacobi_iters), &T, &lo, &hi, &exch);
    if (!m->sharded()) lo = 1 - (int)m->j0, hi = (int)m->g.ny - 1 - (int)m->j0;
    int pad = 0, occ = 0, nwc = 0, nseg = 0;
    lds_geometry8(m->g, lo, hi, persist != 0, &pad, &occ, &nwc, &nseg);
    if (lds_pad) *lds_pad = pad;
    if (wgs_per_cu) *wgs_per_cu = occ;
    if (wave_cols) *wave_cols = nwc;
    if (segments) *segments = nseg;
    return 0;
}

int cfd_get_persist_steals(cfd_model *m, uint64_t *steals) {
    if (!m || !steals) return fail(CFD_EINVAL, "null argument");
    int rc = m->sync();
    if (rc) return rc;
    uint32_t v = 0;
    HIP_TRY(hipMemcpy(&v, m->f.persist + 2, 4, hipMemcpyDeviceToHost));
    *steals = v;
    return 0;
}

int cfd_get_persist_sums(cfd_model *m, uint64_t *blocks) {
    if (!m || !blocks) return fail(CFD_EINVAL, "null argument");
    int rc = m->sync();
    if (rc) return rc;
    uint32_t v = 0;
    HIP_TRY(hipMemcpy(&v, m->f.persist + 3, 4, hipMemcpyDeviceToHost));
    *blocks = v;
    return 0;
}

int cfd_get_sums_launches(cfd_model *m, uint64_t *launches) {
    if (!m || !launches) return fail(CFD_EINVAL, "null argument");
    Ctl c;
    int rc = m->read_ctl(&c);
    if (rc) return rc;
    *launches = c.sums_launches;
    return 0;
}

int cfd_get_sums_bounds(cfd_model *m, uint32_t *state, uint32_t *m0_bits, uint32_t *rm_bits) {
    if (!m || !state || !m0_bits || !rm_bits) return fail(CFD_EINVAL, "null argument");
    Ctl c;
    int rc = m->read_ctl(&c);
    if (rc) return rc;
    const bool on = m->f.sums_track != 0;
    *state = on ? c.sums_state : 0u;
    *m0_bits = on ? c.sums_m0 : 0u;
    *rm_bits = on ? c.sums_rm : 0u;
    return 0;
}

int cfd_get_comm_calls(const cfd_model *m, uint64_t *n) {
    if (!m || !n) return fail(CFD_EINVAL, "null argument");
    *n = m->comm_calls;
    return 0;
}

int cfd_get_recoveries(const cfd_model *m, uint64_t *n) {
    if (!m || !n) return fail(CFD_EINVAL, "null argument");
    *n = m->recoveries;
    return 0;
}

int cfd_get_resident_solves(const cfd_model *m, uint64_t *solves) {
    if (!m || !solves) return fail(CFD_EINVAL, "null argument");
    *solves = m->resident_solves;
    return 0;
}

int cfd_get_resident_geometry(const cfd_model *m, int *br, int *bc, int *tiles, int *wgs) {
    if (!m) return fail(CFD_EINVAL, "null model");
    int v[4] = {0, 0, 0, 0};
    if (!m->resident_mode() || !jacobi_resident_geometry(m->g, &v[0], &v[1], &v[2], &v[3]))
        return fail(CFD_ESTATE, "the model does not take the resident solve");
    if (br) *br = v[0];
    if (bc) *bc = v[1];
    if (tiles) *tiles = v[2];
    if (wgs) *wgs = v[3];
    return 0;
}

int cfd_get_persist_blocks(const cfd_model *m, int *blocks) {
    if (!m || !blocks) return fail(CFD_EINVAL, "null argument");
    *blocks = m->last_persist_blocks;
    return 0;
}

int cfd_plan_slab(uint64_t ny, int n_ranks, int rank, uint64_t *j0, uint64_t *j1) {
    if (n_ranks < 1 || rank < 0 || rank >= n_ranks || !j0 || !j1)
        return fail(CFD_EINVAL, "bad plan_slab arguments");
    plan_slab(ny, n_ranks, rank, j0, j1);
    return 0;
}

int cfd_plan_sweep(int j0, int nyl, int ny, int halo_depth, int it, int iters, int *lo, int *hi,
                   int *exchange) {
    if (halo_depth < 1 || !lo || !hi || !exchange) return fail(CFD_EINVAL, "bad plan_sweep arguments");
    plan_sweep(j0, nyl, ny, halo_depth, it, iters, lo, hi, exchange);
    return 0;
}

int cfd_plan_block(int j0, int nyl, int ny, int halo_depth, int it, int t_max, int iters, int *T,
                   int *out_lo, int *out_hi, int *exchange) {
    if (t_max < 1 || !T || !out_lo || !out_hi || !exchange)
        return fail(CFD_EINVAL, "bad plan_block arguments");
    plan_block(j0, nyl, ny, halo_depth, it, t_max, iters, T, out_lo, out_hi, exchange);
    return 0;
}

int cfd_plan_overlap(int nyl, int halo_depth, int rank, int n_ranks, int lo, int hi, int *out6) {
    if (!out6 || n_ranks < 1 || rank < 0 || rank >= n_ranks) return fail(CFD_EINVAL, "bad plan_overlap arguments");
    return plan_overlap(nyl, halo_depth, rank, n_ranks, lo, hi, out6);
}

int cfd_plan_halo(int kind, int nyl, int depth, int rank, int n_ranks, int *out6) {
    if (kind < 0 || kind > 2 || !out6) return fail(CFD_EINVAL, "bad plan_halo arguments");
    plan_halo(kind, nyl, depth, rank, n_ranks, out6);
    return 0;
}

void cfd_destroy(cfd_model *m) {
    if (!m) return;
    m->destroy();
    delete m;
}

}
```

### cfd-demo_amd/csrc/cfd_model_build.hip

```cpp
#include <algorithm>
#include <cstring>

#include "cfd_model.h"

using namespace cfd;

namespace cfd {

cfd_options read_options() {
    cfd_options o;
    o.sor_fused = env_flag("CFD_SOR_FUSED", true);
    o.mg_partition = env_flag("CFD_MG_PARTITION", true);
    o.spec = env_flag("CFD_SPEC", true);
    o.spec_lag = env_flag("CFD_SPEC_LAG", true);
    o.spec_slabs = env_flag("CFD_SPEC_SLABS", true);
    o.persist = env_int("CFD_PERSIST", -1);
    o.persist_sharded = env_flag("CFD_PERSIST_SHARDED", false);
    o.persist_gate = env_flag("CFD_PERSIST_GATE", false);
    o.resident = env_int("CFD_RESIDENT", -1);
    o.copy_div = env_flag("CFD_COPY_DIV", true);
    o.pred_vec = env_flag("CFD_PRED_VEC", true);
    o.corr_vec = env_flag("CFD_CORR_VEC", true);
    o.corr_head = env_flag("CFD_CORR_HEAD", true);
    o.graph = env_flag("CFD_GRAPH", false);
    o.ckpt = env_flag("CFD_CKPT", true);
    o.fastdiv = env_int("CFD_FASTDIV", kEnvUnset);
    o.resident_div = env_int("CFD_RESIDENT_DIV", kEnvUnset);
    o.pred_div = env_int("CFD_PRED_DIV", kEnvUnset);
    o.tb_kind = env_int("CFD_TB_KIND", kEnvUnset);
    o.temporal = env_int("CFD_TEMPORAL", kEnvUnset);
    o.tb_rows = env_int("CFD_TB_ROWS", kEnvUnset);
    o.tb_bpc = env_int("CFD_TB_BPC", kEnvUnset);
    o.xcd_remap = env_int("CFD_XCD_REMAP", kEnvUnset);
    o.rccl_timeout_s = std::max(1.0, env_double("CFD_RCCL_TIMEOUT_S", 300.0));
    return o;
}

int validate(const cfd_grid *grid, const cfd_params *p) {
    if (!grid || !p) return fail(CFD_EINVAL, "null grid or params");
    if (grid->nx < 16 || grid->nx % 8 != 0)
        return fail(CFD_EINVAL, "nx must be a multiple of 8 and >= 16 (model.rs:541 precondition)");
    if (grid->ny < 4) return fail(CFD_EINVAL, "ny must be >= 4");
    if ((grid->nx + 1) * grid->ny > (1ull << 31))
        return fail(CFD_EINVAL, "grid too large for 32-bit row indexing");
    if (!(grid->lx > 0.f) || !(grid->ly > 0.f)) return fail(CFD_EINVAL, "lx, ly must be > 0");
    if (p->jacobi_iters < 0 || p->jacobi_iters > kMaxSweeps)
        return fail(CFD_EINVAL, "jacobi_iters out of range [0, 4096]");
    if (p->corrector_passes < 0 || p->corrector_passes > kMaxPasses - 1)
        return fail(CFD_EINVAL, "corrector_passes out of range [0, 63]");
    if (p->velocity_scheme != 0 && p->velocity_scheme != 1)
        return fail(CFD_EINVAL, "velocity_scheme must be 0 or 1");
    if (p->inlet_profile != 0 && p->inlet_profile != 1)
        return fail(CFD_EINVAL, "inlet_profile must be 0 or 1");
    if (p->pressure_solver < CFD_SOLVER_JACOBI || p->pressure_solver > CFD_SOLVER_JACOBI_SCRIPT ||
        p->pressure_solver == 3)
        return fail(CFD_EINVAL, "pressure_solver must be 0 (Jacobi), 1 (SOR), 2 (multigrid), "
                                "4 (SOR in the script's order) or 5 (the script's Jacobi)");
    if (p->bc_kind != 0 && p->bc_kind != 1) return fail(CFD_EINVAL, "bc_kind must be 0 or 1");
    return 0;
}

int validate_sharded(const cfd_model *m, const cfd_params *p) {
    if (m->n_ranks > 1 && p->pressure_solver == CFD_SOLVER_SOR_LEX)
        return fail(CFD_EINVAL, "pressure_solver 4 (SOR in the script's order) runs on one domain "
                                "only: sharded models take 0, 1 or 2");
    if (m->n_ranks > 1 && p->pressure_solver == CFD_SOLVER_JACOBI_SCRIPT)
        return fail(CFD_EINVAL, "pressure_solver 5 (the script's Jacobi) runs on one domain only: "
                                "sharded models take 0, 1 or 2");
    if (m->n_ranks <= 1 || p->pressure_solver != CFD_SOLVER_SOR) return 0;
    const int lo = std::max(0, 1 - (int)m->j0);
    const int hi = std::min((int)(m->j1 - m->j0), (int)m->grid.ny - 1 - (int)m->j0);
    if (p->jacobi_iters < 1 || m->g.hg < 2 || !sor_fused_ok((int)m->grid.nx, hi - lo))
        return fail(CFD_EINVAL, "sharded SOR needs >= 1 iteration, halo depth >= 2 and >= 16 "
                                "interior rows per slab (rank " + std::to_string(m->rank) + " has " +
                                    std::to_string(hi - lo) + ", halo depth " +
                                    std::to_string(m->g.hg) + ")");
    return 0;
}

void apply_params(cfd_model *m, const cfd_params *p) {
    m->params = *p;
    m->g.nu = p->viscosity;
    m->g.target_inlet = p->target_inlet_velocity;
    m->g.scheme = p->velocity_scheme;
    m->g.profile = p->inlet_profile;
    m->g.bc_kind = p->bc_kind;
    m->g.tol_enabled = p->tol_enabled ? 1 : 0;
    m->g.p_tol = p->p_tol;
    m->g.jacobi_iters = p->jacobi_iters;
}

void set_sums_track(cfd_model *m) {
    const Geom &g = m->g;
    int e2 = 0;
    const bool pow2 = g.r_dx_sq >= 1.0f && std::frexp(g.r_dx_sq, &e2) == 0.5f;
    m->f.sums_track = env_flag("CFD_JACOBI_SUMS", true) && m->n_ranks == 1 && g.j0 == 0 && g.nyl == g.ny &&
                      m->params.pressure_solver == CFD_SOLVER_JACOBI && !g.tol_enabled &&
                      g.fastdiv == 1 && g.dx_sq == g.dy_sq && g.r_dx_sq == g.r_dy_sq && pow2;
}

}

namespace {

std::mutex g_div_mu;
std::vector<std::pair<uint32_t, int>> g_div_cache;

int division_ok_mask(hipStream_t s, float c, float r, int *mask) {
    uint32_t bits;
    std::memcpy(&bits, &c, 4);
    {
        std::lock_guard<std::mutex> lk(g_div_mu);
        for (auto &e : g_div_cache)
            if (e.first == bits) {
                *mask = e.second;
                return 0;
            }
    }
    unsigned long long *d = nullptr, h[3] = {0, 0, 0};
    HIP_TRY(hipMalloc((void **)&d, 24));
    HIP_TRY(hipMemsetAsync(d, 0, 24, s));
    launch_verify_division(c, r, d, s);
    HIP_TRY(hipGetLastError());
    HIP_TRY(hipMemcpyAsync(h, d, 24, hipMemcpyDeviceToHost, s));
    HIP_TRY(hipStreamSynchronize(s));
    HIP_TRY(hipFree(d));
    *mask = (h[0] == 0 ? 1 : 0) | (h[1] == 0 ? 2 : 0) | (h[2] == 0 ? 4 : 0);
    std::lock_guard<std::mutex> lk(g_div_mu);
    g_div_cache.emplace_back(bits, *mask);
    return 0;
}

int choose_division(hipStream_t s, const cfd_options &opt, Geom &g) {
    g.fastdiv = 0;
    g.res_div = 0;
    if (opt.fastdiv == 0) return 0;
    int m1, m2, m3;
    int rc;
    if ((rc = division_ok_mask(s, g.dx_sq, g.r_dx_sq, &m1)) ||
        (rc = division_ok_mask(s, g.dy_sq, g.r_dy_sq, &m2)) ||
        (rc = division_ok_mask(s, g.denom, g.r_denom, &m3)))
        return rc;
    const int all = m1 & m2 & m3;
    g.fastdiv = (all & 1) ? 1 : (all & 2) ? 2 : 0;
    if (opt.fastdiv == 2 && (all & 2)) g.fastdiv = 2;
    g.res_div = g.fastdiv != 0 ? g.fastdiv : (opt.resident_div == 3 && (all & 4)) ? 3 : 0;
    return 0;
}

int build_model(cfd_model *m, const cfd_grid *grid, const cfd_params *p, int device, int hg) {
    const cfd_options &opt = m->opt;
    m->device = device;
    m->grid = *grid;
    HIP_TRY(hipSetDevice(device));
    HIP_TRY(hipStreamCreateWithFlags(&m->stream, hipStreamNonBlocking));
    HIP_TRY(hipStreamCreateWithFlags(&m->cstream, hipStreamNonBlocking));
    HIP_TRY(hipEventCreateWithFlags(&m->ev_ov0, hipEventDisableTiming));
    HIP_TRY(hipEventCreateWithFlags(&m->ev_ov1, hipEventDisableTiming));
    HIP_TRY(hipEventCreateWithFlags(&m->ev_rhs, hipEventDisableTiming));
    HIP_TRY(hipEventCreateWithFlags(&m->ev_uv, hipEventDisableTiming));
    HIP_TRY(hipEventCreate(&m->ev_step0));
    HIP_TRY(hipEventCreate(&m->ev_step1));
    HIP_TRY(hipEventCreate(&m->ev_prof0));
    HIP_TRY(hipEventCreate(&m->ev_prof1));
    const int nx = (int)grid->nx, ny = (int)grid->ny;
    Geom &g = m->g;
    g.nx = nx;
    g.ny = ny;
    g.j0 = (int)m->j0;
    g.nyl = (int)(m->j1 - m->j0);
    g.hg = hg;
    if ((uint64_t)(g.nyl + 2 * hg + 2 * kGhostUV + 1) * (uint64_t)(nx + 1) * 4u >= (1ull << 31))
        return fail(CFD_EINVAL, "slab too large for 32-bit buffer offsets (2 GiB per field)");
    g.dx = grid->lx / (float)grid->nx;
    g.dy = grid->ly / (float)grid->ny;
    g.ly = grid->ly;
    apply_params(m, p);
    g.dx_sq = g.dx * g.dx;
    g.dy_sq = g.dy * g.dy;
    g.denom = 2.0f / (g.dx * g.dx) + 2.0f / (g.dy * g.dy);
    g.r_dx_sq = 1.0f / g.dx_sq;
    g.r_dy_sq = 1.0f / g.dy_sq;
    g.r_denom = 1.0f / g.denom;
    {
        auto pow2f = [](float c) {
            int e;
            return c > 0.0f && std::isfinite(c) && std::frexp(c, &e) == 0.5f &&
                   std::isnormal(1.0f / c);
        };
        g.r_dx = 1.0f / g.dx;
        g.r_dy = 1.0f / g.dy;
        g.r_dxx = 1.0f / (g.dx * g.dx);
        g.r_dyy = 1.0f / (g.dy * g.dy);
        g.sp_pow2 = pow2f(g.dx) && pow2f(g.dy) && pow2f(g.dx * g.dx) && pow2f(g.dy * g.dy) ? 1 : 0;
        if (opt.fastdiv == 0) g.sp_pow2 = 0;
    }
    {
        int rc0 = choose_division(m->stream, opt, g);
        if (rc0) return rc0;
    }
    g.tb_kind = g.fastdiv == 1 ? 5 : 4;
    g.pred_div = opt.pred_div == 0 ? 0 : 2;
    if (opt.tb_kind != kEnvUnset) {
        const int k = opt.tb_kind;
        if (k != 1 && k != 4 && k != 5) return fail(CFD_EINVAL, "CFD_TB_KIND must be 1, 4 or 5");
        g.tb_kind = k;
    }
    if (g.tb_kind != 5 && (uint64_t)(g.nyl + 2 * g.hg) * (uint64_t)nx * 4u > (1ull << 30))
        g.tb_kind = 1;
    m->t_max = 4;
    {
        const uint64_t jac_ws = 3ull * (uint64_t)(g.nyl + 2 * g.hg) * (uint64_t)nx * 4u;
        if (g.tb_kind == 4 && g.fastdiv == 1 && m->n_ranks == 1 && jac_ws > (256ull << 20))
            m->t_max = 8;
        if (g.tb_kind == 5) m->t_max = 8;
    }
    if (opt.temporal != kEnvUnset) m->t_max = std::max(1, opt.temporal);
    m->t_max = std::min(m->t_max, g.tb_kind == 1 ? 4 : kMaxTemporal);
    g.tb_rows = g.tb_kind == 5 ? 0 : 24;
    if (opt.tb_rows != kEnvUnset) g.tb_rows = std::max(4, std::min(1024, opt.tb_rows));
    g.tb_bpc = 3;
    if (opt.tb_bpc != kEnvUnset) {
        g.tb_bpc = std::max(1, std::min(16, opt.tb_bpc));
        g.tb_rows = 0;
    }
    g.xcd_remap = opt.xcd_remap == 0 ? 0 : 1;
    {
        int ncu = 0;
        if (hipDeviceGetAttribute(&ncu, hipDeviceAttributeMultiprocessorCount, device) != hipSuccess ||
            ncu <= 0)
            ncu = 256;
        g.n_cu = ncu;
    }


    const size_t W = (size_t)nx + 1, nyl = (size_t)g.nyl;
    const size_t u_alloc = round4(m->u_rows_alloc() * W);
    const size_t v_alloc = round4(m->v_rows_alloc() * (size_t)nx);
    const size_t p_n = nyl * nx;
    const size_t pp_n = (nyl + 2 * (size_t)hg) * nx;
    auto zalloc = [&](void **ptr, size_t bytes) -> int {
        HIP_TRY(hipMalloc(ptr, bytes));
        HIP_TRY(hipMemsetAsync(*ptr, 0, bytes, m->stream));
        return 0;
    };
    int rc = 0;
    if ((rc = zalloc((void **)&m->u_all, u_alloc * 4)) || (rc = zalloc((void **)&m->v_all, v_alloc * 4)) ||
        (rc = zalloc((void **)&m->uo_all, u_alloc * 4)) || (rc = zalloc((void **)&m->vo_all, v_alloc * 4)) ||
        (rc = zalloc((void **)&m->us_all, u_alloc * 4)) || (rc = zalloc((void **)&m->vs_all, v_alloc * 4)) ||
        (rc = zalloc((void **)&m->p, p_n * 4)) || (rc = zalloc((void **)&m->rhs, pp_n * 4)) ||
        (rc = zalloc((void **)&m->pp_all[0], pp_n * 4)) || (rc = zalloc((void **)&m->pp_all[1], pp_n * 4)) ||
        (rc = zalloc((void **)&m->mask_u, nyl * W + 16)) || (rc = zalloc((void **)&m->mask_v, (nyl + 1) * nx + 16)) ||
        (rc = zalloc((void **)&m->ctl, sizeof(Ctl))) ||
        (rc = zalloc((void **)&m->slots, kSlotWords * 4)))
        return rc;
    m->ck_segs = {{m->u_all, u_alloc * 4}, {m->v_all, v_alloc * 4}, {m->uo_all, u_alloc * 4},
                  {m->vo_all, v_alloc * 4}, {m->us_all, u_alloc * 4}, {m->vs_all, v_alloc * 4},
                  {m->p, p_n * 4},         {m->rhs, pp_n * 4},        {m->pp_all[0], pp_n * 4},
                  {m->pp_all[1], pp_n * 4}, {m->ctl, sizeof(Ctl)}};
    HIP_TRY(hipHostMalloc((void **)&m->h_nonfinite, 16, hipHostMallocMapped | hipHostMallocCoherent));
    *(volatile uint32_t *)m->h_nonfinite = 0u;
    *(volatile uint32_t *)(m->h_nonfinite + 1) = 0u;
    *(volatile uint32_t *)(m->h_nonfinite + 2) = 0u;
    HIP_TRY(hipHostMalloc((void **)&m->h_res, 4 * cfd_model::kResRing, hipHostMallocDefault));
    for (hipEvent_t &e : m->ev_res) HIP_TRY(hipEventCreateWithFlags(&e, hipEventDisableTiming));
    HIP_TRY(hipHostMalloc((void **)&m->h_spec, 4 * cfd_model::kSpecRing * kMaxTemporal, hipHostMallocDefault));
    for (hipEvent_t &e : m->ev_spec) HIP_TRY(hipEventCreateWithFlags(&e, hipEventDisableTiming));

    std::vector<uint8_t> mu(nyl * W, 0), mv((nyl + 1) * nx, 0);
    std::vector<int32_t> obs;
    if (grid->has_cylinder) {
        for (int j = 0; j < ny; ++j) {
            for (int i = 0; i < nx; ++i) {
                const float x = ((float)i + 0.5f) * g.dx;
                const float y = ((float)j + 0.5f) * g.dy;
                const float ddx = x - grid->cylinder_x;
                const float ddy = y - grid->cylinder_y;
                const float distance = std::sqrt(ddx * ddx + ddy * ddy);
                if (!(distance < grid->cylinder_radius)) continue;
                const long lj = (long)j - (long)m->j0;
                if (lj >= 0 && lj < (long)nyl) {
                    if (i > 0) mu[lj * W + i] = 1;
                    if (i < nx) mu[lj * W + i + 1] = 1;
                }
                if (j > 0 && lj >= 0 && lj <= (long)nyl) mv[lj * nx + i] = 1;
                if (j < ny && lj + 1 >= 0 && lj + 1 <= (long)nyl) mv[(lj + 1) * nx + i] = 1;
                if (lj >= 0 && lj <= (long)nyl) {
                    obs.push_back(i);
                    obs.push_back(j);
                }
            }
        }
    }
    m->h_mask_u = mu;
    m->h_mask_v = mv;
    std::vector<uint8_t> dmu(mu), dmv(mv);
    for (size_t k = 0; k < obs.size(); k += 2) {
        const long oi = obs[k], lj = (long)obs[k + 1] - (long)m->j0;
        if (lj >= 0 && lj < (long)nyl) dmu[lj * W + oi] |= 2;
        if (lj >= 0 && lj <= (long)nyl) dmv[lj * nx + oi] |= 2;
    }
    m->dmask_u = std::move(dmu);
    m->dmask_v = std::move(dmv);
    HIP_TRY(hipMemcpyAsync(m->mask_u, m->dmask_u.data(), m->dmask_u.size(), hipMemcpyHostToDevice,
                           m->stream));
    HIP_TRY(hipMemcpyAsync(m->mask_v, m->dmask_v.data(), m->dmask_v.size(), hipMemcpyHostToDevice,
                           m->stream));
    if (!obs.empty()) {
        HIP_TRY(hipMalloc((void **)&m->obs, obs.size() * 4));
        HIP_TRY(hipMemcpyAsync(m->obs, obs.data(), obs.size() * 4, hipMemcpyHostToDevice, m->stream));
    }

    Fields &f = m->f;
    const size_t uoff = (size_t)kGhostUV * W, voff = (size_t)kGhostUV * nx;
    f.u_alloc_base = m->u_all;
    f.v_alloc_base = m->v_all;
    f.u_old_base = m->uo_all;
    f.v_old_base = m->vo_all;
    f.u_star_base = m->us_all;
    f.v_star_base = m->vs_all;
    f.u_alloc = u_alloc;
    f.v_alloc = v_alloc;
    f.u = m->u_all + uoff;
    f.v = m->v_all + voff;
    f.u_old = m->uo_all + uoff;
    f.v_old = m->vo_all + voff;
    f.u_star = m->us_all + uoff;
    f.v_star = m->vs_all + voff;
    f.p = m->p;
    f.rhs = m->rhs + (size_t)hg * nx;
    f.pp[0] = m->pp_all[0] + (size_t)hg * nx;
    f.pp[1] = m->pp_all[1] + (size_t)hg * nx;
    const std::pair<const float *, const char *> rows16[] = {
        {f.v, "v"}, {f.v_star, "v_star"}, {f.p, "p"}, {f.rhs, "rhs"}, {f.pp[0], "pp[0]"}, {f.pp[1], "pp[1]"}};
    for (const auto &r : rows16)
        if (!aligned16(r.first))
            return fail(CFD_EINVAL, std::string("field ") + r.second + " is not 16-byte aligned");
    f.mask_u = m->mask_u;
    f.mask_v = m->mask_v;
    f.obs = m->obs;
    f.n_obs = (int32_t)(obs.size() / 2);
    f.any_pmask = 0;
    for (uint8_t b : m->h_mask_u) f.any_pmask |= b & 1;
    for (uint8_t b : m->h_mask_v) f.any_pmask |= b & 1;
    f.ctl = m->ctl;
    {
        void *dp = nullptr;
        HIP_TRY(hipHostGetDevicePointer(&dp, m->h_nonfinite, 0));
        f.host_nonfinite = (uint32_t *)dp;
        f.host_progress = m->n_ranks > 1 ? (uint32_t *)dp + 1 : nullptr;
    }
    f.err_slots = m->slots;
    f.red_slots = m->slots + (size_t)kMaxSweeps * kResSlots * kResStride;
    f.vis_slots = f.red_slots + (size_t)4 * kResSlots * kResStride;
    f.persist = m->slots + (size_t)(kMaxSweeps + 16) * kResSlots * kResStride;

    set_sums_track(m);

    Ctl c0;
    std::memset(&c0, 0, sizeof(c0));
    c0.dt = p->dt;
    c0.go[0] = 1;
    HIP_TRY(hipMemcpyAsync(m->ctl, &c0, sizeof(Ctl), hipMemcpyHostToDevice, m->stream));
    HIP_TRY(hipStreamSynchronize(m->stream));
    return 0;
}

}

namespace cfd {

int create_model(const cfd_grid *grid, const cfd_params *params, int device, int n_ranks, int rank,
                 const void *uid, LocalHub *hub, cfd_model **out) {
    if (!out) return fail(CFD_EINVAL, "null out");
    *out = nullptr;
    int rc = validate(grid, params);
    if (rc) return rc;
    if (n_ranks < 1 || rank < 0 || rank >= n_ranks) return fail(CFD_EINVAL, "bad rank/n_ranks");
    if (n_ranks > 1 && params->pressure_solver == CFD_SOLVER_SOR_LEX)
        return fail(CFD_EINVAL, "pressure_solver 4 (SOR in the script's order) runs on one domain "
                                "only: sharded models take 0, 1 or 2");
    if (n_ranks > 1 && params->pressure_solver == CFD_SOLVER_JACOBI_SCRIPT)
        return fail(CFD_EINVAL, "pressure_solver 5 (the script's Jacobi) runs on one domain only: "
                                "sharded models take 0, 1 or 2");
    int ndev = 0;
    if (hipGetDeviceCount(&ndev) != hipSuccess || ndev == 0)
        return fail(CFD_EHIP, "no HIP device available");
    if (device < 0 || device >= ndev) return fail(CFD_EINVAL, "device ordinal out of range");
    cfd_model *m = new cfd_model();
    m->opt = read_options();
    m->persist_on = m->opt.persist != 0;
    m->n_ranks = n_ranks;
    m->rank = rank;
    plan_slab(grid->ny, n_ranks, rank, &m->j0, &m->j1);
    int hg = 1;
    if (n_ranks > 1) {
        uint64_t min_rows = grid->ny / (uint64_t)n_ranks;
        hg = env_int("CFD_HALO_DEPTH", (int)std::max<uint64_t>(kMaxTemporal,
                                                                std::min<uint64_t>(32, min_rows / 32)));
        if (hg < 1) hg = 1;
        if ((uint64_t)hg + 2 > min_rows) hg = (int)(min_rows > 3 ? min_rows - 2 : 1);
        if (min_rows < 4) {
            delete m;
            return fail(CFD_EINVAL, "each slab needs at least 4 rows");
        }
    }
    rc = build_model(m, grid, params, device, hg);
    if (!rc) rc = validate_sharded(m, params);
    if (!rc && n_ranks > 1 && hub) {
        if (hub->n != n_ranks) {
            rc = fail(CFD_EINVAL, "local hub size != n_ranks");
        } else {
            std::lock_guard<std::mutex> lk(hub->mu);
            hub->members[rank] = m;
            m->hub = hub;
        }
    } else if (!rc && n_ranks > 1) {
        ncclUniqueId id;
        std::memcpy(&id, uid, sizeof(id));
        rc = comm_init(m, id, n_ranks, rank);
    }
    if (rc) {
        m->destroy();
        delete m;
        return rc;
    }
    *out = m;
    return 0;
}

}

void cfd_model::destroy() {
    {
        PersistGate &gate = persist_gate(device);
        std::lock_guard<std::mutex> lk(gate.mu);
        if (gate.last == stream) gate.last = nullptr;
    }
    (void)hipSetDevice(device);
    if (stream) (void)hipStreamSynchronize(stream);
    if (comm) ncclCommDestroy(comm);
    comm = nullptr;
    for (hipEvent_t e : ev_res)
        if (e) (void)hipEventDestroy(e);
    if (h_res) (void)hipHostFree(h_res);
    for (hipEvent_t e : ev_spec)
        if (e) (void)hipEventDestroy(e);
    if (h_spec) (void)hipHostFree(h_spec);
    for (void *ptr : {(void *)u_all, (void *)v_all, (void *)uo_all, (void *)vo_all,
                      (void *)us_all, (void *)vs_all, (void *)p, (void *)rhs,
                      (void *)pp_all[0], (void *)pp_all[1], (void *)mask_u, (void *)mask_v,
                      (void *)obs, (void *)ctl, (void *)slots, (void *)vis_buf,
                      (void *)mg_pool, (void *)mg_dev, (void *)lex_pol, (void *)lex_exit,
                      (void *)res64})
        if (ptr) (void)hipFree(ptr);
    if (h_nonfinite) (void)hipHostFree(h_nonfinite);
    if (ck_pool) (void)hipFree(ck_pool);
    if (trc_pool) (void)hipFree(trc_pool);
    if (trc_dens) (void)hipFree(trc_dens);
    if (scr_pool) (void)hipFree(scr_pool);
    if (su_pool) (void)hipFree(su_pool);
    if (su_h) (void)hipHostFree(su_h);
    drop_graph();
    for (hipEvent_t e : ev_pool) (void)hipEventDestroy(e);
    if (ev_step0) (void)hipEventDestroy(ev_step0);
    if (ev_step1) (void)hipEventDestroy(ev_step1);
    if (ev_prof0) (void)hipEventDestroy(ev_prof0);
    if (ev_prof1) (void)hipEventDestroy(ev_prof1);
    if (stream) (void)hipStreamDestroy(stream);
    if (cstream) (void)hipStreamDestroy(cstream);
    if (ev_ov0) (void)hipEventDestroy(ev_ov0);
    if (ev_ov1) (void)hipEventDestroy(ev_ov1);
    if (ev_rhs) (void)hipEventDestroy(ev_rhs);
    if (ev_uv) (void)hipEventDestroy(ev_uv);
}
```

### cfd-demo_amd/csrc/cfd_model_extras.hip

```cpp
#include <cstring>

#include "cfd_model.h"

using namespace cfd;

int cfd_model::trc_release() {
    if (!trc_pool) return 0;
    for (size_t k = 0; k < ck_segs.size(); ++k)
        if (ck_segs[k].ptr == (void *)trc_pool) {
            ck_segs.erase(ck_segs.begin() + (long)k);
            break;
        }
    if (int rc = ck_drop_pool()) return rc;
    HIP_TRY(hipFree(trc_pool));
    trc_pool = nullptr;
    trc = Tracers{};
    return 0;
}

bool cfd_model::scr_in_obstacle(double x, double y) const {
    if (!grid.has_cylinder) return false;
    const double ex = x - (double)grid.cylinder_x, ey = y - (double)grid.cylinder_y;
    return std::sqrt(ex * ex + ey * ey) <= (double)grid.cylinder_radius;
}
int cfd_model::script_build() {
    if (scr_pool) return 0;
    const int nx = g.nx, ny = g.ny;
    const double dx = (double)g.dx, dy = (double)g.dy;
    std::vector<int32_t> iv((size_t)2 * ny + 2 * (ny + 1), 0);
    auto row = [&](int32_t *out, int n, auto inside) -> bool {
        int lo = -1, hi = -1, cnt = 0;
        for (int i = 0; i < n; ++i)
            if (inside(i)) {
                if (lo < 0) lo = i;
                hi = i + 1;
                ++cnt;
            }
        if (cnt && hi - lo != cnt) return false;
        out[0] = cnt ? lo : 0;
        out[1] = cnt ? hi : 0;
        return true;
    };
    bool ok = true;
    for (int j = 0; j < ny && ok; ++j)
        ok = row(&iv[(size_t)2 * j], nx + 1,
                 [&](int i) { return scr_in_obstacle((double)i * dx, ((double)j + 0.5) * dy); });
    for (int j = 0; j <= ny && ok; ++j)
        ok = row(&iv[(size_t)2 * ny + 2 * j], nx,
                 [&](int i) { return scr_in_obstacle(((double)i + 0.5) * dx, (double)j * dy); });
    if (!ok) return fail(CFD_ESTATE, "script step: a row's obstacle faces are not one interval");
    const size_t ib = iv.size() * 4, bytes = ib + (size_t)ny * 4;
    HIP_TRY(hipMalloc((void **)&scr_pool, bytes));
    HIP_TRY(hipMemcpy(scr_pool, iv.data(), ib, hipMemcpyHostToDevice));
    HIP_TRY(hipMemset(scr_pool + ib, 0, (size_t)ny * 4));
    scr.obs_u = (const int32_t *)scr_pool;
    scr.obs_v = scr.obs_u + 2 * ny;
    scr.inlet = (const float *)(scr_pool + ib);
    scr.dx = dx;
    scr.dy = dy;
    scr.dxx = dx * dx;
    scr.dyy = dy * dy;
    scr.nu = (double)g.nu;
    scr.r_dx = 1.0 / scr.dx;
    scr.r_dy = 1.0 / scr.dy;
    scr.r_dxx = 1.0 / scr.dxx;
    scr.r_dyy = 1.0 / scr.dyy;
    scr.fast = exact_pow2(scr.dx) && exact_pow2(scr.dy) && exact_pow2(scr.dxx) && exact_pow2(scr.dyy) ? 1 : 0;
    scr_inlet_h.assign((size_t)ny, 0.0f);
    return 0;
}
int cfd_model::script_prepare(const cfd_script_step *s, ScriptStep *out) {
    if (int rc = script_build()) return rc;
    scr.nu = (double)g.nu;
    if (scr_inlet_profile != s->inlet_profile ||
        std::memcmp(&scr_inlet_v, &s->inlet_velocity, 8) != 0) {
        const int ny = g.ny;
        const double ly = (double)grid.ly, dy = (double)g.dy;
        for (int j = 0; j < ny; ++j) {
            double val = s->inlet_velocity;
            if (s->inlet_profile == CFD_INLET_PARABOLIC) {
                const double y = ((double)j + 0.5) * dy;
                const double center = ly / 2, radius = ly / 2;
                const double t = (y - center) / radius;
                val = s->inlet_velocity * (1 - t * t);
                val = val > 0 ? val : (val != val ? val : 0.0);
            }
            scr_inlet_h[(size_t)j] = (float)val;
        }
        HIP_TRY(hipMemcpyAsync((void *)scr.inlet, scr_inlet_h.data(), (size_t)ny * 4,
                               hipMemcpyHostToDevice, stream));
        scr_inlet_v = s->inlet_velocity;
        scr_inlet_profile = s->inlet_profile;
    }
    *out = scr;
    out->dt = s->dt_sub;
    return 0;
}

extern "C" {

namespace {

constexpr uint64_t kTrcMaxCap = 1ull << 30;

const char *const kTrcOverflowMsg =
    "tracer capacity overflow: an injection of ny tracers did not fit; the list is no longer the "
    "script's until cfd_tracers_enable or cfd_tracers_set";

int trc_read(cfd_model *m, TrcCtl *tc) {
    if (!m) return fail(CFD_EINVAL, "null model");
    if (!m->trc_pool) return fail(CFD_ESTATE, "tracers are not enabled (cfd_tracers_enable)");
    int rc = m->sync();
    if (rc) return rc;
    HIP_TRY(hipMemcpy(tc, m->trc.tc, sizeof(TrcCtl), hipMemcpyDeviceToHost));
    if (tc->overflow) return fail(CFD_ESTATE, kTrcOverflowMsg);
    return 0;
}

int trc_begin_call(cfd_model *m) {
    if (!m) return fail(CFD_EINVAL, "null model");
    if (!m->trc_pool) return fail(CFD_ESTATE, "tracers are not enabled (cfd_tracers_enable)");
    return m->sync();
}

}

int cfd_tracers_enable(cfd_model *m, uint64_t capacity, int inject_interval) {
    if (!m) return fail(CFD_EINVAL, "null model");
    if (m->sharded())
        return fail(CFD_EINVAL, "tracers run on one domain only: a tracer reads u and v rows of "
                                "other slabs");
    const uint64_t ny = (uint64_t)m->g.ny;
    if (capacity < ny || capacity > kTrcMaxCap)
        return fail(CFD_EINVAL, "tracer capacity must be in [ny, 2^30] (ny = " + std::to_string(ny) + ")");
    int rc = m->sync();
    if (rc) return rc;
    if ((rc = m->trc_release())) return rc;
    m->drop_graph();
    const size_t ntiles = (size_t)((capacity + kTrcBlock - 1) / kTrcBlock);
    const size_t head = (256 + 2 * ntiles * 4 + 255) & ~(size_t)255;
    const size_t arr = ((size_t)capacity * 8 + 255) & ~(size_t)255;
    const size_t bytes = head + 6 * arr;
    char *pool = nullptr;
    HIP_TRY(hipMalloc((void **)&pool, bytes));
    m->trc_pool = pool;
    m->trc_bytes = bytes;
    HIP_TRY(hipMemset(pool, 0, bytes));
    Tracers &t = m->trc;
    t.tc = (TrcCtl *)pool;
    t.tile_cnt = (uint32_t *)(pool + 256);
    t.tile_off = t.tile_cnt + ntiles;
    double **arrs[6] = {&t.x0, &t.y0, &t.i0, &t.x1, &t.y1, &t.i1};
    for (int k = 0; k < 6; ++k) *arrs[k] = (double *)(pool + head + (size_t)k * arr);
    t.cap = (uint32_t)capacity;
    t.interval = inject_interval <= 0 ? 100u : (uint32_t)inject_interval;
    t.dx = (double)m->g.dx;
    t.dy = (double)m->g.dy;
    t.lx = (double)m->grid.lx;
    t.ly = (double)m->grid.ly;
    long grid = std::min<long>((long)ntiles, 8l * std::max(1, m->g.n_cu));
    if (const long cap = env_long("CFD_TRACER_WGS", 0); cap >= 1) grid = std::min<long>(grid, cap);
    m->trc_grid = (int)std::max(1l, grid);
    if ((rc = m->ck_drop_pool())) return rc;
    m->ck_segs.push_back({pool, bytes});
    launch_trc_inject(m->g, t, m->stream);
    HIP_TRY(hipGetLastError());
    HIP_TRY(hipStreamSynchronize(m->stream));
    return 0;
}

int cfd_tracers_disable(cfd_model *m) {
    if (!m) return fail(CFD_EINVAL, "null model");
    if (!m->trc_pool) return 0;
    int rc = m->sync();
    if (rc) return rc;
    return m->trc_release();
}

int cfd_tracers_count(cfd_model *m, uint64_t *n) {
    TrcCtl tc;
    int rc = trc_read(m, &tc);
    if (rc) return rc;
    if (n) *n = tc.count;
    return 0;
}

int cfd_tracers_get(cfd_model *m, double *x, double *y, double *initial_y, uint64_t max,
                    uint64_t *n_out) {
    TrcCtl tc;
    int rc = trc_read(m, &tc);
    if (rc) return rc;
    const Tracers &t = m->trc;
    const size_t n = (size_t)std::min<uint64_t>(tc.count, max);
    if (x && n) HIP_TRY(hipMemcpy(x, tc.cur ? t.x1 : t.x0, n * 8, hipMemcpyDeviceToHost));
    if (y && n) HIP_TRY(hipMemcpy(y, tc.cur ? t.y1 : t.y0, n * 8, hipMemcpyDeviceToHost));
    if (initial_y && n) HIP_TRY(hipMemcpy(initial_y, tc.cur ? t.i1 : t.i0, n * 8, hipMemcpyDeviceToHost));
    if (n_out) *n_out = n;
    return 0;
}

int cfd_tracers_set(cfd_model *m, const double *x, const double *y, const double *initial_y,
                    uint64_t n) {
    if (!m) return fail(CFD_EINVAL, "null model");
    if (!m->trc_pool) return fail(CFD_ESTATE, "tracers are not enabled (cfd_tracers_enable)");
    if (n > m->trc.cap) return fail(CFD_EINVAL, "more tracers than the capacity");
    if (n && (!x || !y || !initial_y)) return fail(CFD_EINVAL, "null tracer array");
    for (uint64_t k = 0; k < n; ++k)
        if (!std::isfinite(x[k]) || !std::isfinite(y[k]) || !std::isfinite(initial_y[k]))
            return fail(CFD_EINVAL, "non-finite tracer coordinate at index " + std::to_string(k));
    int rc = m->sync();
    if (rc) return rc;
    const Tracers &t = m->trc;
    if (n) {
        HIP_TRY(hipMemcpy(t.x0, x, (size_t)n * 8, hipMemcpyHostToDevice));
        HIP_TRY(hipMemcpy(t.y0, y, (size_t)n * 8, hipMemcpyHostToDevice));
        HIP_TRY(hipMemcpy(t.i0, initial_y, (size_t)n * 8, hipMemcpyHostToDevice));
    }
    TrcCtl tc{};
    tc.count = (uint32_t)n;
    HIP_TRY(hipMemcpy(t.tc, &tc, sizeof(TrcCtl), hipMemcpyHostToDevice));
    return 0;
}

int cfd_tracers_advance(cfd_model *m, double dt) {
    int rc = trc_begin_call(m);
    if (rc) return rc;
    launch_trc_step(m->g, m->f, m->trc, m->trc_grid, false, dt, m->stream);
    HIP_TRY(hipGetLastError());
    return 0;
}

int cfd_tracers_inject(cfd_model *m) {
    int rc = trc_begin_call(m);
    if (rc) return rc;
    launch_trc_inject(m->g, m->trc, m->stream);
    HIP_TRY(hipGetLastError());
    return 0;
}

int cfd_tracers_density(cfd_model *m, uint32_t *counts_nx_ny) {
    TrcCtl tc;
    int rc = trc_read(m, &tc);
    if (rc) return rc;
    if (!counts_nx_ny) return fail(CFD_EINVAL, "null counts");
    const size_t cells = (size_t)m->g.nx * (size_t)m->g.ny;
    if (!m->trc_dens) HIP_TRY(hipMalloc((void **)&m->trc_dens, cells * 4));
    HIP_TRY(hipMemsetAsync(m->trc_dens, 0, cells * 4, m->stream));
    launch_trc_density(m->g, m->trc, m->trc_grid, m->trc_dens, m->stream);
    HIP_TRY(hipGetLastError());
    HIP_TRY(hipMemcpyAsync(counts_nx_ny, m->trc_dens, cells * 4, hipMemcpyDeviceToHost, m->stream));
    HIP_TRY(hipStreamSynchronize(m->stream));
    return 0;
}

}

namespace cfd {

int script_check(cfd_model *m, const cfd_script_step *s) {
    if (!m) return fail(CFD_EINVAL, "null model");
    if (!s) return fail(CFD_EINVAL, "null cfd_script_step");
    if (m->sharded())
        return fail(CFD_EINVAL, "the script substep runs on one domain only");
    if (m->params.bc_kind != CFD_BC_CHANNEL)
        return fail(CFD_EINVAL, "the script substep has the channel boundary conditions only");
    if (m->params.pressure_solver != CFD_SOLVER_MULTIGRID &&
        m->params.pressure_solver != CFD_SOLVER_SOR_LEX &&
        m->params.pressure_solver != CFD_SOLVER_JACOBI_SCRIPT)
        return fail(CFD_EINVAL, "the script substep needs pressure_solver 2 (multigrid), 4 "
                                "(script-order SOR) or 5 (the script's Jacobi): the others are not "
                                "the script's");
    if (s->scheme != CFD_SCRIPT_FIRST && s->scheme != CFD_SCRIPT_SECOND && s->scheme != CFD_SCRIPT_QUICK)
        return fail(CFD_EINVAL, "script scheme must be 0 (first), 1 (second) or 2 (quick)");
    if (s->inlet_profile != CFD_INLET_UNIFORM && s->inlet_profile != CFD_INLET_PARABOLIC)
        return fail(CFD_EINVAL, "unknown inlet profile");
    if (!std::isfinite(s->dt_sub) || !(s->dt_sub > 0.0))
        return fail(CFD_EINVAL, "dt_sub must be finite and positive");
    if (!std::isfinite(s->inlet_velocity)) return fail(CFD_EINVAL, "inlet_velocity must be finite");
    if (!script_step_ok(m->g, m->f))
        return fail(CFD_EINVAL, "grid too large for the script substep's row loads (2 GiB per field)");
    return 0;
}

}

int cfd_model::script_substep(const cfd_script_step *s) {
    HIP_TRY(hipSetDevice(device));
    if (int rc = invalidate_sums()) return rc;
    if (int rc = ck_begin()) return rc;
    cfd_model *m = this;
    const cfd_script_step st = *s;
    auto run = [m, st]() {
        ScriptStep k;
        if (int rc = m->script_prepare(&st, &k)) return rc;
        launch_script_predict(m->g, m->f, k, st.scheme, m->stream);
        HIP_TRY(hipGetLastError());
        if (int rc = m->enqueue_solve(-1)) return rc;
        launch_script_correct(m->g, m->f, k, m->stream);
        HIP_TRY(hipGetLastError());
        return 0;
    };
    m->ck_record(run);
    return run();
}

extern "C" {

int cfd_script_piso_step(cfd_model *m, const cfd_script_step *s) {
    if (int rc = script_check(m, s)) return rc;
    return m->script_substep(s);
}

int cfd_script_phase(cfd_model *m, int phase, const cfd_script_step *s) {
    if (int rc = script_check(m, s)) return rc;
    if (phase != CFD_SCRIPT_PHASE_PREDICT && phase != CFD_SCRIPT_PHASE_CORRECT)
        return fail(CFD_EINVAL, "unknown script phase");
    HIP_TRY(hipSetDevice(m->device));
    if (int rc = m->invalidate_sums()) return rc;
    ScriptStep k;
    if (int rc = m->script_prepare(s, &k)) return rc;
    if (phase == CFD_SCRIPT_PHASE_PREDICT)
        launch_script_predict(m->g, m->f, k, s->scheme, m->stream);
    else
        launch_script_correct(m->g, m->f, k, m->stream);
    HIP_TRY(hipGetLastError());
    return m->sync();
}

}
```

### cfd-demo_amd/csrc/cfd_model_step.hip

```cpp
#include <cstddef>

#include "cfd_model.h"

using namespace cfd;

namespace {
const float kNaN = std::nanf("");
}

hipEvent_t cfd_model::take_event() {
    if (ev_next == ev_pool.size()) {
        hipEvent_t e;
        (void)hipEventCreate(&e);
        ev_pool.push_back(e);
    }
    return ev_pool[ev_next++];
}

hipEvent_t cfd_model::phase_mark(int ph, bool end, hipStream_t st) {
    if (!(timing && timing_phases)) return nullptr;
    hipEvent_t e = take_event();
    (void)hipEventRecord(e, st ? st : stream);
    if (end) phase_events[ph].back().second = e;
    else phase_events[ph].emplace_back(e, nullptr);
    return e;
}

void cfd_model::begin_solve_timing(int pass, hipEvent_t *e0) {
    *e0 = nullptr;
    if (timing && pass <= 0) {
        *e0 = take_event();
        (void)hipEventRecord(*e0, stream);
    }
}
void cfd_model::end_solve_timing(hipEvent_t e0, uint64_t sweeps, uint64_t launches) {
    if (!e0) return;
    hipEvent_t e1 = take_event();
    (void)hipEventRecord(e1, stream);
    solve_events.emplace_back(e0, e1);
    timed_sweeps += sweeps;
    timed_launches += launches;
}

void cfd_model::pass_head(int pass, float dt_override) {
    if (opt.copy_div) {
        launch_copy_star_div(g, f, pass, dt_override, stream);
    } else {
        launch_copy_star(g, f, pass, stream);
        launch_divergence(g, f, pass, dt_override, stream);
    }
}

int cfd_model::enqueue_piso(float dt_override, bool finish) {
    const bool march = predict_march_ok(g, f);
    phase_mark(0, false);
    if (march && finish && uv_async) {
        launch_predict_march(g, f, dt_override, stream, true, 2, g.nyl - 2);
        HIP_TRY(hipStreamWaitEvent(stream, ev_uv, 0));
        launch_predict_march(g, f, dt_override, stream, false, 0, 4);
        launch_predict_march(g, f, dt_override, stream, false, g.nyl - 4, g.nyl);
    } else if (march)
        launch_predict_march(g, f, dt_override, stream, finish && step_begin_folded);
    else
        launch_predict(g, f, dt_override, opt.pred_vec, stream);
    auto first_divergence = [&](int pass) {
        if (!march) launch_divergence(g, f, pass, dt_override, stream);
        phase_mark(0, true);
    };
    if (finish) {
        first_divergence(host_driven() ? -1 : 0);
        merge_res_allreduce = sharded() && !host_driven();
        int rc = host_driven() ? enqueue_solve_host_driven(nullptr) : enqueue_solve(0);
        merge_res_allreduce = false;
        if (rc) return rc;
        phase_mark(1, false);
        launch_correct_finish(g, f, dt_override, stream);
        phase_mark(1, true);
        HIP_TRY(hipGetLastError());
        return 0;
    }
    if (!host_driven()) {
        first_divergence(0);
        int rc = enqueue_solve(0);
        if (rc) return rc;
        const int passes = params.corrector_passes;
        const bool fuse = !sharded() && passes >= 1 && opt.corr_head && correct_head_ok(g, f);
        auto corrector = [&](int pass) {
            if (fuse)
                launch_correct_head(g, f, pass, dt_override, pass < passes, stream);
            else
                launch_corrector(g, f, pass, dt_override, opt.corr_vec, stream);
        };
        corrector(0);
        const bool spec_slabs = sharded() && g.tol_enabled && spec_slab_ok();
        for (int pass = 1; pass <= passes; ++pass) {
            if (!fuse) pass_head(pass, dt_override);
            rc = enqueue_solve(pass);
            if (rc) return rc;
            corrector(pass);
            if (spec_slabs && spec_converged) break;
        }
    } else {
        first_divergence(-1);
        float res = 0.f;
        int rc = enqueue_solve_host_driven(&res);
        if (rc) return rc;
        launch_corrector(g, f, -1, dt_override, opt.corr_vec, stream);
        for (int pass = 1; pass <= params.corrector_passes; ++pass) {
            pass_head(-1, dt_override);
            rc = enqueue_solve_host_driven(&res);
            if (rc) return rc;
            launch_corrector(g, f, -1, dt_override, opt.corr_vec, stream);
            if (res < params.p_tol) break;
        }
    }
    launch_boundary(g, f, stream);
    HIP_TRY(hipGetLastError());
    return 0;
}

int cfd_model::enqueue_update(bool rec_step) {
    if (rec_step) HIP_TRY(hipEventRecord(ev_step0, stream));
    const bool fused = params.corrector_passes == 0;
    step_begin_folded = fused && predict_march_ok(g, f);
    if (!step_begin_folded) launch_step_begin(g, f, fused ? 0 : 1, stream);
    uv_async = sharded() && overlap && fused && step_begin_folded && g.nyl >= 8;
    int rc;
    if (uv_async) {
        HIP_TRY(hipEventRecord(ev_ov0, stream));
        HIP_TRY(hipStreamWaitEvent(cstream, ev_ov0, 0));
        rc = exchange_uv(cstream);
        if (rc) return rc;
        HIP_TRY(hipEventRecord(ev_uv, cstream));
    } else {
        rc = exchange_uv();
    }
    if (rc) return rc;
    rc = enqueue_piso(kNaN, fused);
    if (rc) return rc;
    if (!fused) launch_step_reduce(g, f, stream);
    if (!fused && f.sums_track) launch_publish_sums_m0(g, f, stream);
    if (sharded()) launch_fold_slots(f.ctl->red, f.red_slots, 4, stream);
    if (sharded() && persist_on && opt.persist_sharded) launch_abort_to_red(f, stream);
    rc = allreduce_max_u32(f.ctl->red, 7);
    if (rc) return rc;
    launch_step_finalize(g, f, stream);
    if (trc_pool) launch_trc_step(g, f, trc, trc_grid, true, 0.0, stream);
    HIP_TRY(hipGetLastError());
    if (rec_step) HIP_TRY(hipEventRecord(ev_step1, stream));
    if (timing) timed_steps++;
    if (rec_step) stepped = true;
    return 0;
}

bool cfd_model::graph_ok() const {
    return opt.graph && !sharded() && !timing && !trc_pool &&
           params.pressure_solver == CFD_SOLVER_JACOBI;
}
void cfd_model::drop_graph() {
    if (step_graph) (void)hipGraphExecDestroy(step_graph);
    step_graph = nullptr;
}
int cfd_model::update_graph(int n) {
    if (!step_graph) {
        const int hc0 = host_cur;
        HIP_TRY(hipStreamBeginCapture(stream, hipStreamCaptureModeThreadLocal));
        int rc = 0;
        capturing = true;
        for (int k = 0; k < graph_steps && !rc; ++k) rc = enqueue_update(false);
        capturing = false;
        hipGraph_t graph = nullptr;
        const hipError_t ce = hipStreamEndCapture(stream, &graph);
        if (rc || ce != hipSuccess) {
            if (graph) (void)hipGraphDestroy(graph);
            host_cur = hc0;
            return rc ? rc : fail(CFD_EHIP, std::string("hipStreamEndCapture: ") + hipGetErrorString(ce));
        }
        const hipError_t ie = hipGraphInstantiate(&step_graph, graph, nullptr, nullptr, 0);
        (void)hipGraphDestroy(graph);
        if (ie != hipSuccess) {
            step_graph = nullptr;
            host_cur = hc0;
            return fail(CFD_EHIP, std::string("hipGraphInstantiate: ") + hipGetErrorString(ie));
        }
        graph_cur_delta = (host_cur - hc0) & 1;
        host_cur = hc0;
    }
    int k = 0;
    for (; k + graph_steps <= n - 1; k += graph_steps) {
        HIP_TRY(hipGraphLaunch(step_graph, stream));
        host_cur = (host_cur + graph_cur_delta) & 1;
    }
    for (; k < n; ++k) {
        int rc = enqueue_update(k == n - 1);
        if (rc) return rc;
    }
    return 0;
}

int cfd_model::abort_allreduce() {
    if (!(sharded() && persist_on && opt.persist_sharded)) return 0;
    launch_abort_to_red(f, stream);
    int rc = allreduce_max_u32(f.ctl->red + 6, 1);
    if (rc) return rc;
    launch_abort_from_red(f, stream);
    HIP_TRY(hipGetLastError());
    return 0;
}

int cfd_model::sync() {
    HIP_TRY(hipSetDevice(device));
    int rc = wait_done(nullptr);
    if (rc) return rc;
    rc = persist_timeout_check(true);
    if (rc) return rc;
    ck_commit();
    return 0;
}
int cfd_model::persist_timeout_check(bool at_sync) {
    if (!h_nonfinite || !*(volatile uint32_t *)(h_nonfinite + 2)) return 0;
    if (!at_sync && sharded()) return 0;
    if (params.pressure_solver == CFD_SOLVER_SOR_LEX) {
        HIP_TRY(hipStreamSynchronize(stream));
        *(volatile uint32_t *)(h_nonfinite + 2) = 0u;
        clear_abort_words();
        clear_res64();
        return fail(CFD_ETIMEOUT, "script-order SOR solve timed out waiting for a workgroup; "
                                  "its result is invalid until cfd_set_state");
    }
    const char *which = last_abort_resident ? "resident tolerance-mode" : "persistent";
    HIP_TRY(hipStreamSynchronize(stream));
    if (cstream) HIP_TRY(hipStreamSynchronize(cstream));
    *(volatile uint32_t *)(h_nonfinite + 2) = 0u;
    persist_on = false;
    resident_off = true;
    if (ck_open) {
        const size_t n_entries = ck_replay.size();
        int rc = recover();
        if (rc) return rc;
        return fail(CFD_ETIMEOUT, std::string(which) + " Jacobi solve timed out waiting for a "
                                  "workgroup; recovered: the state was restored from the "
                                  "model's checkpoint and " + std::to_string(n_entries) +
                                  " call(s) re-run with one launch per block (the state is "
                                  "valid); per-launch solves from now on");
    }
    clear_abort_words();
    return fail(CFD_ETIMEOUT, std::string(which) + " Jacobi solve timed out waiting for a "
                              "workgroup (no checkpoint was open); its result is invalid; "
                              "per-launch solves from now on");
}

bool cfd_model::ckpt_needed() const {
    if (!opt.ckpt || params.pressure_solver != CFD_SOLVER_JACOBI) return false;
    if (persist_on && (sharded() ? opt.persist_sharded : opt.persist > 0)) return true;
    return resident_mode();
}
int cfd_model::ck_begin() {
    if (ck_open || !ckpt_needed()) return 0;
    if (!ck_pool) {
        size_t tot = 0;
        for (const CkSeg &sg : ck_segs) tot += (sg.bytes + 255) & ~(size_t)255;
        HIP_TRY(hipMalloc((void **)&ck_pool, tot));
        ck_bytes = tot;
    }
    size_t off = 0;
    for (const CkSeg &sg : ck_segs) {
        HIP_TRY(hipMemcpyAsync(ck_pool + off, sg.ptr, sg.bytes, hipMemcpyDeviceToDevice, stream));
        off += (sg.bytes + 255) & ~(size_t)255;
    }
    ck_host_cur = host_cur;
    ck_shallow = pp_ghosts_shallow;
    ck_replay.clear();
    ck_open = true;
    return 0;
}
void cfd_model::ck_record(std::function<int()> fn) {
    if (ck_open) ck_replay.push_back(std::move(fn));
}
void cfd_model::ck_commit() {
    ck_open = false;
    ck_replay.clear();
}
int cfd_model::invalidate_sums() {
    HIP_TRY(hipMemsetAsync(&ctl->sums_state, 0, 4, stream));
    return 0;
}
int cfd_model::clear_abort_words() {
    HIP_TRY(hipMemset(f.persist, 0, (size_t)kPersistHeadLines * kPersistFlagStride * 4));
    return 0;
}
int cfd_model::recover() {
    size_t off = 0;
    for (const CkSeg &sg : ck_segs) {
        HIP_TRY(hipMemcpy(sg.ptr, ck_pool + off, sg.bytes, hipMemcpyDeviceToDevice));
        off += (sg.bytes + 255) & ~(size_t)255;
    }
    HIP_TRY(hipMemset(f.err_slots, 0, (size_t)kMaxSweeps * kResSlots * kResStride * 4));
    int rc = clear_abort_words();
    if (rc) return rc;
    rc = clear_res64();
    if (rc) return rc;
    *(volatile uint32_t *)h_nonfinite = 0u;
    host_cur = ck_host_cur;
    pp_ghosts_shallow = ck_shallow;
    ++recoveries;
    std::vector<std::function<int()>> replay;
    replay.swap(ck_replay);
    ck_open = false;
    const bool tm = timing;
    timing = false;
    for (auto &fn : replay) {
        rc = fn();
        if (rc) break;
    }
    timing = tm;
    if (rc) return rc;
    rc = wait_done(nullptr);
    if (rc) return rc;
    if (*(volatile uint32_t *)(h_nonfinite + 2))
        return fail(CFD_ETIMEOUT, "the re-run after a solve timeout timed out");
    return 0;
}

int cfd_model::ck_drop_pool() {
    if (ck_pool) HIP_TRY(hipFree(ck_pool));
    ck_pool = nullptr;
    ck_bytes = 0;
    return 0;
}

int cfd_model::read_ctl(Ctl *out) {
    int rc = sync();
    if (rc) return rc;
    HIP_TRY(hipMemcpy(out, f.ctl, offsetof(Ctl, go), hipMemcpyDeviceToHost));
    return 0;
}
```

### cfd-demo_amd/csrc/cfd_predict_march.hip

```cpp
#include "cfd_device.h"
#include "cfd_predict.h"

namespace cfd {
namespace {

#ifndef CFD_PM_WPE
#define CFD_PM_WPE 3
#endif
#ifndef CFD_PM_USTORE
#define CFD_PM_USTORE 0
#endif
#ifndef CFD_PM_ROWS_FO
#define CFD_PM_ROWS_FO 8
#endif
#ifndef CFD_PM_PD
#define CFD_PM_PD 1
#endif

template <int C>
struct MAcc {
    const float (&u)[6][8];
    const float (&v)[6][8];
    int q;
    __device__ __forceinline__ float U(int di, int dj) const { return u[C + dj][q + 2 + di]; }
    __device__ __forceinline__ float V(int di, int dj) const { return v[C + dj][q + 2 + di]; }
};

template <int SCHEME, int SP, bool MASK, int R>
struct PredMarch {
    static constexpr int PD = CFD_PM_PD;
    static constexpr int D = PD + 5;

    float UQ[D][4];
    float VQ[D][4];
    float UB[D], VB[D];
    float vs[4];
    uint32_t rmax;
    const Geom *g;
    Fields f;
    __amdgpu_buffer_rsrc_t rs_u, rs_v, rs_us, rs_vs;
    int vo;
    int i0, c, nch;
    bool st_lane;
    int kb, r0, r1, glo, u_hi, v_hi, W;
    float dt;

    __device__ __forceinline__ void ld_u(float (&d)[4], int row) const {
        row = row < -kGhostUV ? -kGhostUV : (row > g->nyl + kGhostUV - 1 ? g->nyl + kGhostUV - 1 : row);
        const u32x4 x = __builtin_amdgcn_raw_buffer_load_b128(rs_u, vo, (row + kGhostUV) * W * 4, 0);
        d[0] = __uint_as_float(x.x); d[1] = __uint_as_float(x.y);
        d[2] = __uint_as_float(x.z); d[3] = __uint_as_float(x.w);
    }
    __device__ __forceinline__ void ld_v(float (&d)[4], int row) const {
        row = row < -kGhostUV ? -kGhostUV : (row > g->nyl + kGhostUV ? g->nyl + kGhostUV : row);
        const u32x4 x = __builtin_amdgcn_raw_buffer_load_b128(rs_v, vo, (row + kGhostUV) * g->nx * 4, 0);
        d[0] = __uint_as_float(x.x); d[1] = __uint_as_float(x.y);
        d[2] = __uint_as_float(x.z); d[3] = __uint_as_float(x.w);
    }

    __device__ __forceinline__ float ld_b(__amdgpu_buffer_rsrc_t rs, int row, int pitch, int hi) const {
        row = row < -kGhostUV ? -kGhostUV : (row > hi ? hi : row);
        return __uint_as_float(__builtin_amdgcn_raw_buffer_load_b32(rs, 0, (row + kGhostUV) * pitch * 4, 0));
    }
    __device__ __forceinline__ void ld_rows(int t, int slot) {
        ld_u(UQ[slot], kb - 2 + t);
        ld_v(VQ[slot], kb - 1 + t);
        UB[slot] = ld_b(rs_us, kb - 2 + t, W, g->nyl + kGhostUV - 1);
        VB[slot] = ld_b(rs_vs, kb - 1 + t, g->nx, g->nyl + kGhostUV);
    }

    template <int T_, bool GEN, bool INT>
    __device__ __forceinline__ void step(int t) {
        constexpr bool I = INT && !GEN;
        const int k = kb + t;
        const int nx = g->nx;
        Fields ff = f;
        if (!MASK) ff.any_pmask = 0;
        float ux[6][8], vx[6][8];
#pragma unroll
        for (int r = 0; r < 6; ++r)
#pragma unroll
            for (int x = 0; x < 8; ++x) ux[r][x] = vx[r][x] = 0.0f;
#pragma unroll
        for (int r = 0; r < 5; ++r)
#pragma unroll
            for (int x = 0; x < 4; ++x) ux[r][2 + x] = UQ[(T_ + r) % D][x];
#pragma unroll
        for (int r = 1; r < 6; ++r)
#pragma unroll
            for (int x = 0; x < 4; ++x) vx[r][2 + x] = VQ[(T_ + r - 1) % D][x];
        ux[2][0] = from_left(ux[2][4]);
        ux[2][1] = from_left(ux[2][5]);
        ux[2][6] = from_right(ux[2][2]);
        ux[2][7] = from_right(ux[2][3]);
        ux[3][6] = from_right(ux[3][2]);
        vx[2][1] = from_left(vx[2][5]);
        vx[3][0] = from_left(vx[3][4]);
        vx[3][1] = from_left(vx[3][5]);
        vx[3][6] = from_right(vx[3][2]);
        vx[3][7] = from_right(vx[3][3]);
        const float ub = UB[(T_ + 2) % D], vb = VB[(T_ + 2) % D];
        ld_rows(t + D, T_ % D);

        const int rv = k + 1;
        float vn[4];
        if (!GEN || (rv >= glo && rv <= v_hi)) {
#pragma unroll
            for (int q = 0; q < 4; ++q)
                vn[q] = v_pred_val<SCHEME, SP, I>(*g, ff, dt, min(i0 + q, nx - 1), rv,
                                               MAcc<3>{ux, vx, q});
            if (c == 0) vn[0] = vb;
            if (st_lane && c < nch && (!GEN || t > 0 || r0 == 0))
                *reinterpret_cast<float4 *>(f.v_star + (long)rv * nx + i0) =
                    make_float4(vn[0], vn[1], vn[2], vn[3]);
        } else {
            const float4 a = c < nch ? *reinterpret_cast<const float4 *>(f.v_star + (long)rv * nx + i0)
                                     : make_float4(0.f, 0.f, 0.f, 0.f);
            vn[0] = a.x; vn[1] = a.y; vn[2] = a.z; vn[3] = a.w;
        }
        if (!GEN || t > 0) {
            float us[4];
            const long ku = (long)k * W + i0;
            const bool upred = !GEN || (k >= glo && k <= u_hi);
            if (upred) {
#pragma unroll
                for (int q = 0; q < 4; ++q)
                    us[q] = u_pred_val<SCHEME, SP, I>(*g, ff, dt, min(i0 + q, nx), k, MAcc<2>{ux, vx, q});
                if (c == 0) us[0] = ub;
            } else if (c <= nch) {
                const f4u a = *reinterpret_cast<const f4u *>(f.u_star + ku);
                us[0] = a.x; us[1] = a.y; us[2] = a.z; us[3] = a.w;
            } else {
                us[0] = us[1] = us[2] = us[3] = 0.0f;
            }
            const float east = from_right(us[0]);
            if (st_lane) {
                if (c < nch) {
                    if (upred) {
                        if (CFD_PM_USTORE == 0) {
                            *reinterpret_cast<f4u *>(f.u_star + ku) = (f4u){us[0], us[1], us[2], us[3]};
                        } else {
                            f.u_star[ku] = us[0];
                            f.u_star[ku + 1] = us[1];
                            f.u_star[ku + 2] = us[2];
                            f.u_star[ku + 3] = us[3];
                        }
                    }
                    const float4 rh = div4<SP>(*g, us[0], us[1], us[2], us[3], east,
                                               make_float4(vs[0], vs[1], vs[2], vs[3]),
                                               make_float4(vn[0], vn[1], vn[2], vn[3]), dt);
                    *reinterpret_cast<float4 *>(f.rhs + (long)k * nx + i0) = rh;
                    if (f.sums_track)
                        rmax = max(max(rmax, max(abs_bits(rh.x), abs_bits(rh.y))),
                                   max(abs_bits(rh.z), abs_bits(rh.w)));
                } else if (c == nch && upred) {
                    f.u_star[ku] = us[0];
                }
            }
        }
#pragma unroll
        for (int q = 0; q < 4; ++q) vs[q] = vn[q];
    }

    template <int J, bool GEN, int OFF>
    __device__ __forceinline__ void group(int base) {
        if constexpr (J < D) {
            step<(OFF + J) % D, GEN>(base + J);
            group<J + 1, GEN, OFF>(base);
        }
    }

    template <int T, bool INT>
    __device__ __forceinline__ void steps() {
        if constexpr (T <= R) {
            step<T % D, (T < 2 || T == R), INT>(T);
            steps<T + 1, INT>();
        }
    }
    template <bool INT>
    __device__ __forceinline__ void run() {
#pragma unroll
        for (int t = 0; t < D; ++t) ld_rows(t, t);
        steps<0, INT>();
    }
};

template <int SCHEME, int SP, bool MASK, int R>
__global__ __launch_bounds__(kBlock, CFD_PM_WPE) void k_predict_march(Geom g, Fields f, float dt_override,
                                                          int glo, int u_hi, int v_hi, int nwc,
                                                          int nseg, int set_inlet, int row_lo,
                                                          int row_hi) {
    if (set_inlet && blockIdx.x == 0 && threadIdx.x == 0) {
        Ctl *c = f.ctl;
        const uint32_t st = c->step;
        c->inlet = st < 100u ? ((float)st / 100.0f) * g.target_inlet : g.target_inlet;
        c->go[0] = 1;
    }
    if (f.sums_track && blockIdx.x == 0 && threadIdx.x == 0 && row_lo == 0 && row_hi == g.nyl &&
        f.ctl->sums_state == 1u) {
        atomicMax(&f.ctl->sums_rm, __float_as_uint(kSumsRLim));
        f.ctl->sums_state = 2u;
    }
    PredMarch<SCHEME, SP, MASK, R> m;
    const int wave = __builtin_amdgcn_readfirstlane((int)threadIdx.x >> 6);
    const int lane = (int)threadIdx.x & 63;
    const int bid = xcd_block(g);
    const int wc = bid % nwc;
    const int seg = (bid / nwc) * (kBlock / 64) + wave;
    if (seg >= nseg) return;
    const int nx = g.nx;
    m.r0 = row_lo + min(seg * R, row_hi - row_lo - R);
    m.r1 = m.r0 + R;
    m.g = &g;
    m.f = f;
    m.W = nx + 1;
    m.nch = nx / 4;
    m.c = wc * 62 - 1 + lane;
    const bool in_dom = m.c >= 0 && m.c <= m.nch;
    m.i0 = in_dom ? 4 * m.c : 0;
    m.st_lane = in_dom && lane >= 1 && lane <= 62;
    m.vo = in_dom ? 4 * m.i0 : 0x7FFF0000;
    m.rs_u = __builtin_amdgcn_make_buffer_rsrc(f.u_alloc_base, 0, (int)(f.u_alloc * 4), 0x00020000);
    m.rs_v = __builtin_amdgcn_make_buffer_rsrc(f.v_alloc_base, 0, (int)(f.v_alloc * 4), 0x00020000);
    m.rs_us = __builtin_amdgcn_make_buffer_rsrc(f.u_star_base, 0, (int)(f.u_alloc * 4), 0x00020000);
    m.rs_vs = __builtin_amdgcn_make_buffer_rsrc(f.v_star_base, 0, (int)(f.v_alloc * 4), 0x00020000);
    m.glo = glo;
    m.u_hi = u_hi;
    m.v_hi = v_hi;
    m.kb = m.r0 - 1;
    m.dt = dt_of(f.ctl, dt_override);
#pragma unroll
    for (int q = 0; q < 4; ++q) m.vs[q] = 0.0f;
    m.rmax = 0u;
    const int c_lo = wc * 62 - 1, c_hi = wc * 62 + 62;
    const bool interior = 4 * c_lo >= 3 && 4 * c_hi + 3 <= nx - 3 &&
                          g.j0 + m.r0 + 1 >= 2 && g.j0 + m.r1 - 2 <= g.ny - 3;
    if (SCHEME == 1 && interior)
        m.template run<true>();
    else
        m.template run<false>();
    if (f.sums_track) raise_bits_bound(&f.ctl->sums_rm, m.rmax, __float_as_uint(kSumsRLim));
}

}

bool predict_march_ok(const Geom &g, const Fields &f) {
    return g.pred_div == 2 && g.nx % 4 == 0 && g.nx >= 8 && g.nyl >= 4 && aligned16(f.v) &&
           aligned16(f.v_star) && aligned16(f.rhs) && (uint64_t)f.u_alloc * 4u < (1ull << 31) &&
           (uint64_t)f.v_alloc * 4u < (1ull << 31);
}

void launch_predict_march(const Geom &g, const Fields &f, float dt_override, hipStream_t s,
                          bool set_inlet, int row_lo, int row_hi) {
    if (row_hi < 0) row_hi = g.nyl;
    const int glo = (g.j0 > 1 ? g.j0 : 1) - g.j0;
    const int u_hi = ((g.j0 + g.nyl - 1) < (g.ny - 2) ? (g.j0 + g.nyl - 1) : (g.ny - 2)) - g.j0;
    const int v_hi = ((g.j0 + g.nyl) < (g.ny - 1) ? (g.j0 + g.nyl) : (g.ny - 1)) - g.j0;
    const int big = g.scheme == 0 ? CFD_PM_ROWS_FO : 8;
    const int span = row_hi - row_lo;
    const int rows = span >= big ? big : (span >= 8 ? 8 : 4);
    const int nwc = cdiv(g.nx / 4 + 1, 62);
    const int nseg = cdiv(row_hi - row_lo, rows);
    const dim3 grid(nwc * cdiv(nseg, kBlock / 64));
#define CFD_LAUNCH_PM(SC, SPV, MK, R)                                                              \
    hipLaunchKernelGGL((k_predict_march<SC, SPV, MK, R>), grid, dim3(kBlock), 0, s, g, f, dt_override, \
                       glo, u_hi, v_hi, nwc, nseg, set_inlet ? 1 : 0, row_lo, row_hi)
#define CFD_LAUNCH_PM3(SC, SPV, MK)                                         \
    if (CFD_PM_ROWS_FO != 8 && SC == 0 && rows == CFD_PM_ROWS_FO)           \
        CFD_LAUNCH_PM(SC, SPV, MK, (SC == 0 ? CFD_PM_ROWS_FO : 8));          \
    else if (rows == 8) CFD_LAUNCH_PM(SC, SPV, MK, 8); else CFD_LAUNCH_PM(SC, SPV, MK, 4)
#define CFD_LAUNCH_PM2(SC, SPV) \
    if (f.any_pmask) { CFD_LAUNCH_PM3(SC, SPV, true); } else { CFD_LAUNCH_PM3(SC, SPV, false); }
    if (g.scheme == 0) {
        if (g.sp_pow2) { CFD_LAUNCH_PM2(0, 1); } else { CFD_LAUNCH_PM2(0, 0); }
    } else {
        if (g.sp_pow2) { CFD_LAUNCH_PM2(1, 1); } else { CFD_LAUNCH_PM2(1, 0); }
    }
#undef CFD_LAUNCH_PM3
#undef CFD_LAUNCH_PM2
#undef CFD_LAUNCH_PM
}

}
```

Before: 2832 billion.

## Fuse predictor recompute into corrector march and defer u_star/v_star materialization

Adds a fused PISO path for the Jacobi solver. The first march kernel computes only the RHS without storing u_star/v_star. A second finish-march kernel recomputes the predictor in registers and applies the velocity and pressure correction, writing new u/v into the old buffers, which are then swapped. Materializing u_star/v_star is deferred to a lazy kernel that runs only when an API path needs them. This trades recomputation for less memory traffic and fewer kernel launches, at the cost of extra state tracking for graphs, checkpoints and buffer swapping.

New measurement: 2912 billion, median of 6. +2.8%, better.

```diff
diff --git a/cfd-demo_amd/csrc/cfd_correct.h b/cfd-demo_amd/csrc/cfd_correct.h
--- a/cfd-demo_amd/csrc/cfd_correct.h
+++ b/cfd-demo_amd/csrc/cfd_correct.h
@@ -21,6 +21,17 @@
     o.y = v_corr<SP>(g, vs.y, pt.y, pb.y, dt);
     o.z = v_corr<SP>(g, vs.z, pt.z, pb.z, dt);
     o.w = v_corr<SP>(g, vs.w, pt.w, pb.w, dt);
+}
+
+template <int SP>
+__device__ __forceinline__ float cf_u_face(const Geom &g, float inlet, float dt, int i, int j,
+                                           float ustar, float p_right, float p_left) {
+    const int nx = g.nx;
+    if (j == 0) return 0.0f;
+    if (j == g.ny - 1) return (g.bc_kind == 1 && i > 0 && i < nx) ? inlet : 0.0f;
+    if (i == 0) return g.bc_kind == 0 ? inlet_value(g, inlet, j) : 0.0f;
+    if (i == nx) return g.bc_kind == 0 ? u_corr<SP>(g, ustar, p_right, p_left, dt, nx) : 0.0f;
+    return u_corr<SP>(g, ustar, p_right, p_left, dt, i);
 }
 
 __device__ __forceinline__ float4 add4(float4 a, const float4 &b) {
diff --git a/cfd-demo_amd/csrc/cfd_correct.hip b/cfd-demo_amd/csrc/cfd_correct.hip
--- a/cfd-demo_amd/csrc/cfd_correct.hip
+++ b/cfd-demo_amd/csrc/cfd_correct.hip
@@ -202,17 +202,6 @@
 
 
 template <int SP>
-__device__ __forceinline__ float cf_u_face(const Geom &g, float inlet, float dt, int i, int j,
-                                           float ustar, float p_right, float p_left) {
-    const int nx = g.nx;
-    if (j == 0) return 0.0f;
-    if (j == g.ny - 1) return (g.bc_kind == 1 && i > 0 && i < nx) ? inlet : 0.0f;
-    if (i == 0) return g.bc_kind == 0 ? inlet_value(g, inlet, j) : 0.0f;
-    if (i == nx) return g.bc_kind == 0 ? u_corr<SP>(g, ustar, p_right, p_left, dt, nx) : 0.0f;
-    return u_corr<SP>(g, ustar, p_right, p_left, dt, i);
-}
-
-template <int SP>
 __device__ __forceinline__ void cf4_row(const Geom &g, const Fields &f, const float *__restrict__ pp,
                                         float inlet, float dt, int i0, int lj, const float4 &pc,
                                         const float4 &pb, float &du, float &dv, float &mu,
diff --git a/cfd-demo_amd/csrc/cfd_internal.h b/cfd-demo_amd/csrc/cfd_internal.h
--- a/cfd-demo_amd/csrc/cfd_internal.h
+++ b/cfd-demo_amd/csrc/cfd_internal.h
@@ -50,6 +50,7 @@
     int32_t go[kMaxPasses + 1];
     uint32_t err[kMaxSweeps];
     double last_p64;
+    float star_dt;
 };
 
 constexpr int kRes64Stride = 8;
@@ -109,8 +110,10 @@
 void launch_v_predictor(const Geom &g, const Fields &f, float dt_override, hipStream_t s);
 void launch_predict(const Geom &g, const Fields &f, float dt_override, bool vec, hipStream_t s);
 bool predict_march_ok(const Geom &g, const Fields &f);
+int predict_march_workgroups(const Geom &g);
 void launch_predict_march(const Geom &g, const Fields &f, float dt_override, hipStream_t s,
-                          bool set_inlet = false, int row_lo = 0, int row_hi = -1);
+                          bool set_inlet = false, int row_lo = 0, int row_hi = -1, int mode = 0,
+                          bool star = false);
 void launch_divergence(const Geom &g, const Fields &f, int pass, float dt_override,
                        hipStream_t s);
 void launch_jacobi_sweep(const Geom &g, const Fields &f, int pass, int it, int row_lo,
diff --git a/cfd-demo_amd/csrc/cfd_model.h b/cfd-demo_amd/csrc/cfd_model.h
--- a/cfd-demo_amd/csrc/cfd_model.h
+++ b/cfd-demo_amd/csrc/cfd_model.h
@@ -115,6 +115,7 @@
     bool graph = false;
     bool ckpt = true;
     int fastdiv = cfd::kEnvUnset;
+    int uv_fused = cfd::kEnvUnset;
     int resident_div = cfd::kEnvUnset;
     int pred_div = cfd::kEnvUnset;
     int tb_kind = cfd::kEnvUnset;
@@ -198,6 +199,8 @@
     bool stepped = false;
     hipGraphExec_t step_graph = nullptr;
     int graph_cur_delta = 0;
+    int uv_flip = 0, graph_uv_flip = 0, graph_uv_delta = 0, ck_uv_flip = 0;
+    bool star_lazy = false, ck_star_lazy = false;
     int graph_steps = 4;
     struct CkSeg {
         void *ptr;
@@ -315,6 +318,9 @@
     void pass_head(int pass, float dt_override);
     int enqueue_piso(float dt_override, bool finish = false);
     int enqueue_update(bool rec_step = true);
+    bool uv_fused_ok() const;
+    void swap_uv();
+    int need_star();
     bool graph_ok() const;
     void drop_graph();
     int update_graph(int n);
diff --git a/cfd-demo_amd/csrc/cfd_model_abi.hip b/cfd-demo_amd/csrc/cfd_model_abi.hip
--- a/cfd-demo_amd/csrc/cfd_model_abi.hip
+++ b/cfd-demo_amd/csrc/cfd_model_abi.hip
@@ -150,6 +150,7 @@
 int cfd_piso_step(cfd_model *m, float dt_sub) {
     if (!m) return fail(CFD_EINVAL, "null model");
     HIP_TRY(hipSetDevice(m->device));
+    if (int rc = m->need_star()) return rc;
     if (int rc = m->invalidate_sums()) return rc;
     if (int rc = m->ck_begin()) return rc;
     auto run = [m, dt_sub]() {
@@ -187,6 +188,7 @@
 int cfd_run_phase(cfd_model *m, int phase, float dt_sub) {
     if (!m) return fail(CFD_EINVAL, "null model");
     HIP_TRY(hipSetDevice(m->device));
+    if (int rc = m->need_star()) return rc;
     if (int rc = m->invalidate_sums()) return rc;
     switch (phase) {
     case CFD_PHASE_U_PREDICTOR: {
@@ -215,6 +217,8 @@
     int rc = validate(&m->grid, p);
     if (rc) return rc;
     rc = validate_sharded(m, p);
+    if (rc) return rc;
+    rc = m->need_star();
     if (rc) return rc;
     rc = m->sync();
     if (rc) return rc;
@@ -331,7 +335,9 @@
 int cfd_get_state(cfd_model *m, cfd_state *st) {
     if (!m || !st) return fail(CFD_EINVAL, "null argument");
     Ctl c;
-    int rc = m->read_ctl(&c);
+    int rc = m->need_star();
+    if (rc) return rc;
+    rc = m->read_ctl(&c);
     if (rc) return rc;
     const size_t W = (size_t)m->g.nx + 1, nx = (size_t)m->g.nx, nyl = (size_t)m->g.nyl;
     if (st->u) HIP_TRY(hipMemcpy(st->u, m->f.u, nyl * W * 4, hipMemcpyDeviceToHost));
@@ -354,7 +360,9 @@
 int cfd_set_state(cfd_model *m, const cfd_state *st) {
     if (!m || !st) return fail(CFD_EINVAL, "null argument");
     Ctl c;
-    int rc = m->read_ctl(&c);
+    int rc = m->need_star();
+    if (rc) return rc;
+    rc = m->read_ctl(&c);
     if (rc) return rc;
     const size_t W = (size_t)m->g.nx + 1, nx = (size_t)m->g.nx, nyl = (size_t)m->g.nyl;
     if (st->u) HIP_TRY(hipMemcpy(m->f.u, st->u, nyl * W * 4, hipMemcpyHostToDevice));
diff --git a/cfd-demo_amd/csrc/cfd_model_build.hip b/cfd-demo_amd/csrc/cfd_model_build.hip
--- a/cfd-demo_amd/csrc/cfd_model_build.hip
+++ b/cfd-demo_amd/csrc/cfd_model_build.hip
@@ -22,6 +22,7 @@
     o.pred_vec = env_flag("CFD_PRED_VEC", true);
     o.corr_vec = env_flag("CFD_CORR_VEC", true);
     o.corr_head = env_flag("CFD_CORR_HEAD", true);
+    o.uv_fused = env_int("CFD_UV_FUSED", kEnvUnset);
     o.graph = env_flag("CFD_GRAPH", false);
     o.ckpt = env_flag("CFD_CKPT", true);
     o.fastdiv = env_int("CFD_FASTDIV", kEnvUnset);
diff --git a/cfd-demo_amd/csrc/cfd_model_extras.hip b/cfd-demo_amd/csrc/cfd_model_extras.hip
--- a/cfd-demo_amd/csrc/cfd_model_extras.hip
+++ b/cfd-demo_amd/csrc/cfd_model_extras.hip
@@ -286,6 +286,7 @@
 
 int cfd_model::script_substep(const cfd_script_step *s) {
     HIP_TRY(hipSetDevice(device));
+    if (int rc = need_star()) return rc;
     if (int rc = invalidate_sums()) return rc;
     if (int rc = ck_begin()) return rc;
     cfd_model *m = this;
@@ -316,6 +317,7 @@
     if (phase != CFD_SCRIPT_PHASE_PREDICT && phase != CFD_SCRIPT_PHASE_CORRECT)
         return fail(CFD_EINVAL, "unknown script phase");
     HIP_TRY(hipSetDevice(m->device));
+    if (int rc = m->need_star()) return rc;
     if (int rc = m->invalidate_sums()) return rc;
     ScriptStep k;
     if (int rc = m->script_prepare(s, &k)) return rc;
diff --git a/cfd-demo_amd/csrc/cfd_model_step.hip b/cfd-demo_amd/csrc/cfd_model_step.hip
--- a/cfd-demo_amd/csrc/cfd_model_step.hip
+++ b/cfd-demo_amd/csrc/cfd_model_step.hip
@@ -51,9 +51,53 @@
     }
 }
 
+bool cfd_model::uv_fused_ok() const {
+    if (opt.uv_fused == 0 || sharded() || host_driven() ||
+        params.pressure_solver != CFD_SOLVER_JACOBI || !predict_march_ok(g, f))
+        return false;
+    if (opt.uv_fused != kEnvUnset) return true;
+    return g.scheme == 0 && predict_march_workgroups(g) >= 4 * g.n_cu;
+}
+void cfd_model::swap_uv() {
+    std::swap(f.u, f.u_old);
+    std::swap(f.v, f.v_old);
+    std::swap(f.u_alloc_base, f.u_old_base);
+    std::swap(f.v_alloc_base, f.v_old_base);
+    uv_flip ^= 1;
+}
+int cfd_model::need_star() {
+    if (!star_lazy) return 0;
+    HIP_TRY(hipSetDevice(device));
+    Fields fm = f;
+    fm.u = f.u_old;
+    fm.v = f.v_old;
+    fm.u_alloc_base = f.u_old_base;
+    fm.v_alloc_base = f.v_old_base;
+    fm.sums_track = 0;
+    launch_predict_march(g, fm, kNaN, stream, false, 0, -1, 0, true);
+    HIP_TRY(hipGetLastError());
+    star_lazy = false;
+    return 0;
+}
+
 int cfd_model::enqueue_piso(float dt_override, bool finish) {
     const bool march = predict_march_ok(g, f);
+    const bool uvf = finish && uv_fused_ok();
+    if (!uvf)
+        if (int rc = need_star()) return rc;
     phase_mark(0, false);
+    if (uvf) {
+        launch_predict_march(g, f, dt_override, stream, step_begin_folded, 0, -1, 1);
+        phase_mark(0, true);
+        if (int rc = enqueue_solve(0)) return rc;
+        phase_mark(1, false);
+        launch_predict_march(g, f, dt_override, stream, false, 0, -1, 2);
+        phase_mark(1, true);
+        HIP_TRY(hipGetLastError());
+        swap_uv();
+        star_lazy = true;
+        return 0;
+    }
     if (march && finish && uv_async) {
         launch_predict_march(g, f, dt_override, stream, true, 2, g.nyl - 2);
         HIP_TRY(hipStreamWaitEvent(stream, ev_uv, 0));
@@ -163,7 +207,8 @@
 }
 int cfd_model::update_graph(int n) {
     if (!step_graph) {
-        const int hc0 = host_cur;
+        const int hc0 = host_cur, fl0 = uv_flip;
+        const bool sl0 = star_lazy;
         HIP_TRY(hipStreamBeginCapture(stream, hipStreamCaptureModeThreadLocal));
         int rc = 0;
         capturing = true;
@@ -174,6 +219,8 @@
         if (rc || ce != hipSuccess) {
             if (graph) (void)hipGraphDestroy(graph);
             host_cur = hc0;
+            if (uv_flip != fl0) swap_uv();
+            star_lazy = sl0;
             return rc ? rc : fail(CFD_EHIP, std::string("hipStreamEndCapture: ") + hipGetErrorString(ce));
         }
         const hipError_t ie = hipGraphInstantiate(&step_graph, graph, nullptr, nullptr, 0);
@@ -181,15 +228,28 @@
         if (ie != hipSuccess) {
             step_graph = nullptr;
             host_cur = hc0;
+            if (uv_flip != fl0) swap_uv();
+            star_lazy = sl0;
             return fail(CFD_EHIP, std::string("hipGraphInstantiate: ") + hipGetErrorString(ie));
         }
         graph_cur_delta = (host_cur - hc0) & 1;
         host_cur = hc0;
+        graph_uv_flip = fl0;
+        graph_uv_delta = uv_flip ^ fl0;
+        if (uv_flip != fl0) swap_uv();
+        star_lazy = sl0;
     }
     int k = 0;
-    for (; k + graph_steps <= n - 1; k += graph_steps) {
+    if (uv_flip != graph_uv_flip && n > 1) {
+        int rc = enqueue_update(false);
+        if (rc) return rc;
+        k = 1;
+    }
+    for (; uv_flip == graph_uv_flip && k + graph_steps <= n - 1; k += graph_steps) {
         HIP_TRY(hipGraphLaunch(step_graph, stream));
         host_cur = (host_cur + graph_cur_delta) & 1;
+        if (graph_uv_delta) swap_uv();
+        if (uv_fused_ok() && params.corrector_passes == 0) star_lazy = true;
     }
     for (; k < n; ++k) {
         int rc = enqueue_update(k == n - 1);
@@ -270,6 +330,8 @@
     }
     ck_host_cur = host_cur;
     ck_shallow = pp_ghosts_shallow;
+    ck_uv_flip = uv_flip;
+    ck_star_lazy = star_lazy;
     ck_replay.clear();
     ck_open = true;
     return 0;
@@ -303,6 +365,8 @@
     *(volatile uint32_t *)h_nonfinite = 0u;
     host_cur = ck_host_cur;
     pp_ghosts_shallow = ck_shallow;
+    if (uv_flip != ck_uv_flip) swap_uv();
+    star_lazy = ck_star_lazy;
     ++recoveries;
     std::vector<std::function<int()>> replay;
     replay.swap(ck_replay);
diff --git a/cfd-demo_amd/csrc/cfd_predict_march.hip b/cfd-demo_amd/csrc/cfd_predict_march.hip
--- a/cfd-demo_amd/csrc/cfd_predict_march.hip
+++ b/cfd-demo_amd/csrc/cfd_predict_march.hip
@@ -1,3 +1,4 @@
+#include "cfd_correct.h"
 #include "cfd_device.h"
 #include "cfd_predict.h"
 
@@ -26,7 +27,7 @@
     __device__ __forceinline__ float V(int di, int dj) const { return v[C + dj][q + 2 + di]; }
 };
 
-template <int SCHEME, int SP, bool MASK, int R>
+template <int SCHEME, int SP, bool MASK, int R, int MODE>
 struct PredMarch {
     static constexpr int PD = CFD_PM_PD;
     static constexpr int D = PD + 5;
@@ -44,6 +45,75 @@
     bool st_lane;
     int kb, r0, r1, glo, u_hi, v_hi, W;
     float dt;
+    bool no_rhs;
+    float PB[4], PC[4], PN[4], QC[4], QN[4];
+    const float *pp;
+    float inlet, du, dv, mu, mv;
+    uint32_t pm;
+    bool bad, ld_p;
+    int own_lo;
+
+    __device__ __forceinline__ void ld_p4(float (&d)[4], const float *base, int row) const {
+        if (ld_p && row >= 0 && row < g->nyl) {
+            const float4 a = *reinterpret_cast<const float4 *>(base + (long)row * g->nx + i0);
+            d[0] = a.x; d[1] = a.y; d[2] = a.z; d[3] = a.w;
+        } else {
+            d[0] = d[1] = d[2] = d[3] = 0.0f;
+        }
+    }
+
+    __device__ __forceinline__ void fin_row(int k, const float (&us)[4], const float (&uo)[5],
+                                            const float (&vold)[4], float pl) {
+        const int nx = g->nx;
+        const int j = g->j0 + k;
+        const long rp = (long)k * nx + i0, ku = (long)k * W + i0;
+        if (i0 == 0) pl = 0.0f;
+        float n0 = cf_u_face<SP>(*g, inlet, dt, i0, j, us[0], PC[0], pl);
+        float n1 = cf_u_face<SP>(*g, inlet, dt, i0 + 1, j, us[1], PC[1], PC[0]);
+        float n2 = cf_u_face<SP>(*g, inlet, dt, i0 + 2, j, us[2], PC[2], PC[1]);
+        float n3 = cf_u_face<SP>(*g, inlet, dt, i0 + 3, j, us[3], PC[3], PC[2]);
+        if (f.n_obs > 0) {
+            if (f.mask_u[ku] & 2) n0 = 0.0f;
+            if (f.mask_u[ku + 1] & 2) n1 = 0.0f;
+            if (f.mask_u[ku + 2] & 2) n2 = 0.0f;
+            if (f.mask_u[ku + 3] & 2) n3 = 0.0f;
+        }
+        *reinterpret_cast<f4u *>(f.u_old + ku) = (f4u){n0, n1, n2, n3};
+        du = fmaxf(fmaxf(fmaxf(du, fabsf(n0 - uo[0])), fmaxf(fabsf(n1 - uo[1]), fabsf(n2 - uo[2]))),
+                   fabsf(n3 - uo[3]));
+        mu = fmaxf(fmaxf(fmaxf(mu, fabsf(n0)), fmaxf(fabsf(n1), fabsf(n2))), fabsf(n3));
+        bad |= nonfinite(n0) || nonfinite(n1) || nonfinite(n2) || nonfinite(n3);
+        if (i0 + 4 == nx) {
+            float n4 = cf_u_face<SP>(*g, inlet, dt, nx, j, us[3], PC[3], PC[2]);
+            if (f.n_obs > 0 && (f.mask_u[ku + 4] & 2)) n4 = 0.0f;
+            f.u_old[ku + 4] = n4;
+            du = fmaxf(du, fabsf(n4 - uo[4]));
+            mu = fmaxf(mu, fabsf(n4));
+            bad |= nonfinite(n4);
+        }
+        const float4 pc = make_float4(PC[0], PC[1], PC[2], PC[3]);
+        float4 nv = make_float4(0.f, 0.f, 0.f, 0.f);
+        if (j != 0 && j != g->ny)
+            v_corr4<SP>(*g, make_float4(vs[0], vs[1], vs[2], vs[3]), pc,
+                        make_float4(PB[0], PB[1], PB[2], PB[3]), dt, nv);
+        fin_v(rp, nv, vold);
+        *reinterpret_cast<float4 *>(f.p + rp) = add4(make_float4(QC[0], QC[1], QC[2], QC[3]), pc);
+        if (f.sums_track)
+            pm = max(max(pm, max(abs_bits(pc.x), abs_bits(pc.y))), max(abs_bits(pc.z), abs_bits(pc.w)));
+    }
+    __device__ __forceinline__ void fin_v(long rp, float4 nv, const float (&vold)[4]) {
+        if (f.n_obs > 0) {
+            if (f.mask_v[rp] & 2) nv.x = 0.0f;
+            if (f.mask_v[rp + 1] & 2) nv.y = 0.0f;
+            if (f.mask_v[rp + 2] & 2) nv.z = 0.0f;
+            if (f.mask_v[rp + 3] & 2) nv.w = 0.0f;
+        }
+        *reinterpret_cast<float4 *>(f.v_old + rp) = nv;
+        dv = fmaxf(fmaxf(fmaxf(dv, fabsf(nv.x - vold[0])), fmaxf(fabsf(nv.y - vold[1]), fabsf(nv.z - vold[2]))),
+                   fabsf(nv.w - vold[3]));
+        mv = fmaxf(fmaxf(fmaxf(mv, fabsf(nv.x)), fmaxf(fabsf(nv.y), fabsf(nv.z))), fabsf(nv.w));
+        bad |= nonfinite(nv.x) || nonfinite(nv.y) || nonfinite(nv.z) || nonfinite(nv.w);
+    }
 
     __device__ __forceinline__ void ld_u(float (&d)[4], int row) const {
         row = row < -kGhostUV ? -kGhostUV : (row > g->nyl + kGhostUV - 1 ? g->nyl + kGhostUV - 1 : row);
@@ -65,7 +135,7 @@
     __device__ __forceinline__ void ld_rows(int t, int slot) {
         ld_u(UQ[slot], kb - 2 + t);
         ld_v(VQ[slot], kb - 1 + t);
-        UB[slot] = ld_b(rs_us, kb - 2 + t, W, g->nyl + kGhostUV - 1);
+        UB[slot] = MODE == 2 ? 0.0f : ld_b(rs_us, kb - 2 + t, W, g->nyl + kGhostUV - 1);
         VB[slot] = ld_b(rs_vs, kb - 1 + t, g->nx, g->nyl + kGhostUV);
     }
 
@@ -101,6 +171,13 @@
         vx[3][7] = from_right(vx[3][3]);
         const float ub = UB[(T_ + 2) % D], vb = VB[(T_ + 2) % D];
         ld_rows(t + D, T_ % D);
+        float pl = 0.0f;
+        if (MODE == 2) {
+            if (GEN && t == 0) ld_p4(PC, pp, k);
+            ld_p4(PN, pp, k + 1 < r1 ? k + 1 : -1);
+            ld_p4(QN, f.p, k + 1 < r1 ? k + 1 : -1);
+            pl = from_left(PC[3]);
+        }
 
         const int rv = k + 1;
         float vn[4];
@@ -110,9 +187,11 @@
                 vn[q] = v_pred_val<SCHEME, SP, I>(*g, ff, dt, min(i0 + q, nx - 1), rv,
                                                MAcc<3>{ux, vx, q});
             if (c == 0) vn[0] = vb;
-            if (st_lane && c < nch && (!GEN || t > 0 || r0 == 0))
+            if (MODE == 0 && st_lane && c < nch && (!GEN || t > 0 || r0 == 0))
                 *reinterpret_cast<float4 *>(f.v_star + (long)rv * nx + i0) =
                     make_float4(vn[0], vn[1], vn[2], vn[3]);
+        } else if (MODE == 2) {
+            vn[0] = vn[1] = vn[2] = vn[3] = 0.0f;
         } else {
             const float4 a = c < nch ? *reinterpret_cast<const float4 *>(f.v_star + (long)rv * nx + i0)
                                      : make_float4(0.f, 0.f, 0.f, 0.f);
@@ -127,16 +206,26 @@
                 for (int q = 0; q < 4; ++q)
                     us[q] = u_pred_val<SCHEME, SP, I>(*g, ff, dt, min(i0 + q, nx), k, MAcc<2>{ux, vx, q});
                 if (c == 0) us[0] = ub;
-            } else if (c <= nch) {
+            } else if (MODE != 2 && c <= nch) {
                 const f4u a = *reinterpret_cast<const f4u *>(f.u_star + ku);
                 us[0] = a.x; us[1] = a.y; us[2] = a.z; us[3] = a.w;
             } else {
                 us[0] = us[1] = us[2] = us[3] = 0.0f;
             }
-            const float east = from_right(us[0]);
-            if (st_lane) {
+            const float east = MODE == 2 ? 0.0f : from_right(us[0]);
+            if (MODE == 2) {
+                if (st_lane && c < nch && k >= own_lo) {
+                    const float uo[5] = {ux[2][2], ux[2][3], ux[2][4], ux[2][5], ux[2][6]};
+                    const float vold[4] = {vx[2][2], vx[2][3], vx[2][4], vx[2][5]};
+                    fin_row(k, us, uo, vold, pl);
+                    if (GEN && t == R && r1 == g->nyl) {
+                        const float vtop[4] = {vx[3][2], vx[3][3], vx[3][4], vx[3][5]};
+                        fin_v((long)(k + 1) * nx + i0, make_float4(0.f, 0.f, 0.f, 0.f), vtop);
+                    }
+                }
+            } else if (st_lane) {
                 if (c < nch) {
-                    if (upred) {
+                    if (MODE == 0 && upred) {
                         if (CFD_PM_USTORE == 0) {
                             *reinterpret_cast<f4u *>(f.u_star + ku) = (f4u){us[0], us[1], us[2], us[3]};
                         } else {
@@ -146,20 +235,30 @@
                             f.u_star[ku + 3] = us[3];
                         }
                     }
-                    const float4 rh = div4<SP>(*g, us[0], us[1], us[2], us[3], east,
-                                               make_float4(vs[0], vs[1], vs[2], vs[3]),
-                                               make_float4(vn[0], vn[1], vn[2], vn[3]), dt);
-                    *reinterpret_cast<float4 *>(f.rhs + (long)k * nx + i0) = rh;
-                    if (f.sums_track)
-                        rmax = max(max(rmax, max(abs_bits(rh.x), abs_bits(rh.y))),
-                                   max(abs_bits(rh.z), abs_bits(rh.w)));
-                } else if (c == nch && upred) {
+                    if (MODE == 1 || !no_rhs) {
+                        const float4 rh = div4<SP>(*g, us[0], us[1], us[2], us[3], east,
+                                                   make_float4(vs[0], vs[1], vs[2], vs[3]),
+                                                   make_float4(vn[0], vn[1], vn[2], vn[3]), dt);
+                        *reinterpret_cast<float4 *>(f.rhs + (long)k * nx + i0) = rh;
+                        if (f.sums_track)
+                            rmax = max(max(rmax, max(abs_bits(rh.x), abs_bits(rh.y))),
+                                       max(abs_bits(rh.z), abs_bits(rh.w)));
+                    }
+                } else if (MODE == 0 && c == nch && upred) {
                     f.u_star[ku] = us[0];
                 }
             }
         }
 #pragma unroll
         for (int q = 0; q < 4; ++q) vs[q] = vn[q];
+        if (MODE == 2) {
+#pragma unroll
+            for (int q = 0; q < 4; ++q) {
+                PB[q] = PC[q];
+                PC[q] = PN[q];
+                QC[q] = QN[q];
+            }
+        }
     }
 
     template <int J, bool GEN, int OFF>
@@ -185,29 +284,29 @@
     }
 };
 
-template <int SCHEME, int SP, bool MASK, int R>
-__global__ __launch_bounds__(kBlock, CFD_PM_WPE) void k_predict_march(Geom g, Fields f, float dt_override,
-                                                          int glo, int u_hi, int v_hi, int nwc,
-                                                          int nseg, int set_inlet, int row_lo,
-                                                          int row_hi) {
+template <int SCHEME, int SP, bool MASK, int R, int MODE>
+__device__ __forceinline__ void march_body(Geom g, Fields f, float dt_override, int glo,
+                                           int u_hi, int v_hi, int nwc, int nseg, int set_inlet,
+                                           int row_lo, int row_hi, int star) {
     if (set_inlet && blockIdx.x == 0 && threadIdx.x == 0) {
         Ctl *c = f.ctl;
         const uint32_t st = c->step;
         c->inlet = st < 100u ? ((float)st / 100.0f) * g.target_inlet : g.target_inlet;
         c->go[0] = 1;
     }
-    if (f.sums_track && blockIdx.x == 0 && threadIdx.x == 0 && row_lo == 0 && row_hi == g.nyl &&
-        f.ctl->sums_state == 1u) {
+    if (MODE != 2 && f.sums_track && blockIdx.x == 0 && threadIdx.x == 0 && row_lo == 0 &&
+        row_hi == g.nyl && f.ctl->sums_state == 1u) {
         atomicMax(&f.ctl->sums_rm, __float_as_uint(kSumsRLim));
         f.ctl->sums_state = 2u;
     }
-    PredMarch<SCHEME, SP, MASK, R> m;
+    PredMarch<SCHEME, SP, MASK, R, MODE> m;
     const int wave = __builtin_amdgcn_readfirstlane((int)threadIdx.x >> 6);
     const int lane = (int)threadIdx.x & 63;
     const int bid = xcd_block(g);
     const int wc = bid % nwc;
     const int seg = (bid / nwc) * (kBlock / 64) + wave;
-    if (seg >= nseg) return;
+    const bool idle = seg >= nseg;
+    if (MODE != 2 && idle) return;
     const int nx = g.nx;
     m.r0 = row_lo + min(seg * R, row_hi - row_lo - R);
     m.r1 = m.r0 + R;
@@ -228,20 +327,59 @@
     m.u_hi = u_hi;
     m.v_hi = v_hi;
     m.kb = m.r0 - 1;
-    m.dt = dt_of(f.ctl, dt_override);
+    m.dt = star ? f.ctl->star_dt : dt_of(f.ctl, dt_override);
+    m.no_rhs = star != 0;
+    m.own_lo = row_lo + seg * R;
+    m.ld_p = m.c >= 0 && m.c < m.nch;
+    m.du = m.dv = m.mu = m.mv = 0.0f;
+    m.pm = 0u;
+    m.bad = false;
+    if (MODE == 2) {
+        m.inlet = f.ctl->inlet;
+        m.pp = f.ctl->cur ? f.pp[1] : f.pp[0];
+#pragma unroll
+        for (int q = 0; q < 4; ++q) m.PB[q] = m.PC[q] = m.PN[q] = m.QC[q] = m.QN[q] = 0.0f;
+    }
 #pragma unroll
     for (int q = 0; q < 4; ++q) m.vs[q] = 0.0f;
     m.rmax = 0u;
     const int c_lo = wc * 62 - 1, c_hi = wc * 62 + 62;
     const bool interior = 4 * c_lo >= 3 && 4 * c_hi + 3 <= nx - 3 &&
                           g.j0 + m.r0 + 1 >= 2 && g.j0 + m.r1 - 2 <= g.ny - 3;
-    if (SCHEME == 1 && interior)
+    if (MODE == 2 && idle) {
+    } else if (SCHEME == 1 && interior)
         m.template run<true>();
     else
         m.template run<false>();
+    if (MODE == 2) {
+        if (blockIdx.x == 0 && threadIdx.x == 0) f.ctl->star_dt = m.dt;
+        flag_nonfinite(f.ctl, m.bad);
+        if (f.sums_track) publish_sums_m0_bound(g, f.ctl, m.pm);
+        publish_step_maxima(f, bid, m.du, m.dv, m.mu, m.mv);
+        return;
+    }
     if (f.sums_track) raise_bits_bound(&f.ctl->sums_rm, m.rmax, __float_as_uint(kSumsRLim));
 }
 
+template <int SCHEME, int SP, bool MASK, int R, bool RHS_ONLY>
+__global__ __launch_bounds__(kBlock, CFD_PM_WPE) void k_predict_march(Geom g, Fields f, float dt_override,
+                                                          int glo, int u_hi, int v_hi, int nwc,
+                                                          int nseg, int set_inlet, int row_lo,
+                                                          int row_hi, int star) {
+    march_body<SCHEME, SP, MASK, R, RHS_ONLY ? 1 : 0>(g, f, dt_override, glo, u_hi, v_hi, nwc, nseg,
+                                                      set_inlet, row_lo, row_hi, star);
+}
+template <int SCHEME, int SP, bool MASK, int R>
+__global__ __launch_bounds__(kBlock, SCHEME == 1 ? 2 : CFD_PM_WPE) void k_finish_march(
+    Geom g, Fields f, float dt_override, int glo, int u_hi, int v_hi, int nwc, int nseg, int row_lo,
+    int row_hi) {
+    march_body<SCHEME, SP, MASK, R, 2>(g, f, dt_override, glo, u_hi, v_hi, nwc, nseg, 0, row_lo, row_hi, 0);
+}
+
+}
+
+int predict_march_workgroups(const Geom &g) {
+    return cdiv(g.nx / 4 + 1, 62) * cdiv(cdiv(g.nyl, 8), kBlock / 64);
 }
 
 bool predict_march_ok(const Geom &g, const Fields &f) {
@@ -251,20 +389,29 @@
 }
 
 void launch_predict_march(const Geom &g, const Fields &f, float dt_override, hipStream_t s,
-                          bool set_inlet, int row_lo, int row_hi) {
+                          bool set_inlet, int row_lo, int row_hi, int mode, bool star) {
     if (row_hi < 0) row_hi = g.nyl;
     const int glo = (g.j0 > 1 ? g.j0 : 1) - g.j0;
     const int u_hi = ((g.j0 + g.nyl - 1) < (g.ny - 2) ? (g.j0 + g.nyl - 1) : (g.ny - 2)) - g.j0;
     const int v_hi = ((g.j0 + g.nyl) < (g.ny - 1) ? (g.j0 + g.nyl) : (g.ny - 1)) - g.j0;
     const int big = g.scheme == 0 ? CFD_PM_ROWS_FO : 8;
     const int span = row_hi - row_lo;
-    const int rows = span >= big ? big : (span >= 8 ? 8 : 4);
+    const int rows = (mode == 2 && g.scheme == 1) ? 4 : span >= big ? big : (span >= 8 ? 8 : 4);
     const int nwc = cdiv(g.nx / 4 + 1, 62);
     const int nseg = cdiv(row_hi - row_lo, rows);
     const dim3 grid(nwc * cdiv(nseg, kBlock / 64));
-#define CFD_LAUNCH_PM(SC, SPV, MK, R)                                                              \
-    hipLaunchKernelGGL((k_predict_march<SC, SPV, MK, R>), grid, dim3(kBlock), 0, s, g, f, dt_override, \
-                       glo, u_hi, v_hi, nwc, nseg, set_inlet ? 1 : 0, row_lo, row_hi)
+#define CFD_LAUNCH_PMM(SC, SPV, MK, R, RO)                                                    \
+    hipLaunchKernelGGL((k_predict_march<SC, SPV, MK, R, RO>), grid, dim3(kBlock), 0, s, g, f,  \
+                       dt_override, glo, u_hi, v_hi, nwc, nseg, set_inlet ? 1 : 0, row_lo, row_hi, \
+                       star ? 1 : 0)
+#define CFD_LAUNCH_PM(SC, SPV, MK, R)                                                          \
+    do {                                                                                       \
+        if (mode == 2)                                                                         \
+            hipLaunchKernelGGL((k_finish_march<SC, SPV, MK, (SC == 1 ? 4 : R)>), grid, dim3(kBlock), 0, s, g, f, \
+                               dt_override, glo, u_hi, v_hi, nwc, nseg, row_lo, row_hi);       \
+        else if (mode == 1) CFD_LAUNCH_PMM(SC, SPV, MK, R, true);                              \
+        else CFD_LAUNCH_PMM(SC, SPV, MK, R, false);                                            \
+    } while (0)
 #define CFD_LAUNCH_PM3(SC, SPV, MK)                                         \
     if (CFD_PM_ROWS_FO != 8 && SC == 0 && rows == CFD_PM_ROWS_FO)           \
         CFD_LAUNCH_PM(SC, SPV, MK, (SC == 0 ? CFD_PM_ROWS_FO : 8));          \
@@ -279,6 +426,7 @@
 #undef CFD_LAUNCH_PM3
 #undef CFD_LAUNCH_PM2
 #undef CFD_LAUNCH_PM
-}
-
-}
+#undef CFD_LAUNCH_PMM
+}
+
+}
```
